# ChaissonLab/LRA

Hardware: AMD Instinct MI355X
Metric: aligned Gbp/s, 30 kb ONT vs GRCh38 (MapRead_lowacc end to end incl. SAM text), per job (higher is better)
Workload: dtype int32

## Files before the change

### lra_amd/csrc/sdp.h

```cpp
#pragma once
#include "common.h"
#include <vector>

namespace lra_sdp {

constexpr int LV = 18;
constexpr uint32_t NONE = 0xFFFFFFFFu;
constexpr int MAXALN = 16;
constexpr int PEN_TAB_WG = 4096, PEN_TAB_WAVE = 2048;
constexpr int TRACE_CAP = 2560;

struct PwlTab { long long stops[25]; float slope[25], inter[25]; int c1, c2; };

struct Ent { long long val; int b; float v; };
struct Node {
  uint32_t dBase;
  uint32_t nD, nE;
  int32_t last;
  uint32_t sTop, nBlk;
  uint32_t stkOff, blkOff;
  uint32_t stkCap, blkCap;
  long long eLast;
};

struct ReadArena { uint64_t base; uint32_t entOff, apOff, stkOff, visOff, blkPair, poolPair, poolPairs, edOff; };

struct PtArgs {
  uint64_t nc;
  const uint64_t* cluster_off; const uint64_t* c_start; const uint32_t* c_count; const int32_t* c_strand;
  const uint32_t* q; const uint32_t* t; const int32_t* len;
  const uint32_t* clusRead; const uint64_t* clusFragOff; const uint64_t* clusPtOff; const uint64_t* fragOff; const uint64_t* ptOff;
  const float* rate_in; float rate; int single;
  uint32_t* fq; uint32_t* ft; int32_t* flen; uint32_t* fcl; uint32_t* fai; float* fval; uint32_t* fprevNode; uint32_t* fprevInd; uint8_t* fflags;
  uint8_t* used; uint8_t* fstrand;
  const uint32_t* qe; const uint32_t* te; uint32_t* fqe; uint32_t* fte;
  uint64_t* key1; uint32_t* pay1; uint32_t* iq; uint32_t* it; uint8_t* ifl; uint32_t* ifr; uint32_t* ptRead;
};

struct BuildArgs {
  int r0, n;
  const uint32_t* order;
  const uint64_t* ptOff;
  const uint32_t* hq; const uint32_t* ht; const uint8_t* hfl; const uint32_t* h2; const uint64_t* key3; const uint32_t* pay3;
  uint32_t* scratch;
  uint32_t* cntEntries; uint32_t* cntNodes; uint32_t* cntD; uint32_t* cntV; uint32_t* cntRC;
  const ReadArena* ra;
  uint32_t* status;
  unsigned long long* stat;
};

struct ProcArgs {
  int r0, n;
  const uint32_t* order;
  const uint64_t* ptOff; const uint64_t* fragOff;
  const uint8_t* hfl; const uint32_t* hfr;
  const int32_t* flen; float* fval; uint32_t* fprevNode; uint32_t* fprevInd; uint8_t* fflags;
  const float* rate_in; float rate;
  const ReadArena* ra; uint32_t* poolUsed;
  uint32_t* status;
  PwlTab pwl;
  const short* penTab; int penN;
  int dbg;
  int wgNoRing;
  char* wgScratch; const uint64_t* wgOff;
  unsigned long long* stat;
};

struct TraceArgs {
  int r0, n, numAln, single; float alnthres;
  int boxes, globalK; const uint32_t* fqe; const uint32_t* fte; const int32_t* numAnchors; int32_t* chainNum;
  const uint64_t* fragOff; const uint64_t* read_off;
  const uint32_t* fq; const uint32_t* ft; const int32_t* flen; const uint32_t* fcl; const uint32_t* fai;
  const float* fval; const uint32_t* fpred; const uint8_t* fflags; const uint32_t* opay;
  uint8_t* used;
  const ReadArena* ra;
  uint32_t* nChains; uint64_t* chainStart; uint32_t* chainLen; uint32_t* chainBox; float* chainValue;
  uint32_t* ccl; uint32_t* can; uint8_t* clink; uint32_t* cq; uint32_t* ct; int32_t* clen; uint8_t* cstrand; const uint8_t* fstrand;
  const uint32_t* status;
};

namespace {
__device__ __forceinline__ void wave_sync() {
  __builtin_amdgcn_fence(__ATOMIC_RELEASE, "workgroup");
  __builtin_amdgcn_wave_barrier();
  __builtin_amdgcn_fence(__ATOMIC_ACQUIRE, "workgroup");
}
__device__ __forceinline__ int wave_incl_scan(int v, int lane) {
  (void)lane;
#define LRA_DPP_ADD(ctrl_, rmask_) v += __builtin_amdgcn_update_dpp(0, v, (ctrl_), (rmask_), 0xf, false)
  LRA_DPP_ADD(0x111, 0xf);
  LRA_DPP_ADD(0x112, 0xf);
  LRA_DPP_ADD(0x114, 0xf);
  LRA_DPP_ADD(0x118, 0xf);
  LRA_DPP_ADD(0x142, 0xa);
  LRA_DPP_ADD(0x143, 0xc);
#undef LRA_DPP_ADD
  return v;
}
__device__ __host__ inline uint32_t al256(uint64_t x) { return (uint32_t)((x + 255) & ~(uint64_t)255); }
__device__ __forceinline__ char* arena_ptr(uint64_t addr) { return (char*)(__attribute__((address_space(1))) char*)addr; }
}

#pragma GCC visibility push(hidden)
struct StatBuf {
  unsigned long long* d = nullptr;
  StatBuf() = default;
  StatBuf(const StatBuf&) = delete;
  StatBuf& operator=(const StatBuf&) = delete;
  ~StatBuf() { release(); }
  void alloc(size_t words, hipStream_t st) { release(); if (hipMalloc((void**)&d, words * 8) != hipSuccess) d = nullptr; else (void)hipMemsetAsync(d, 0, words * 8, st); }
  void release() { if (d) (void)hipFree(d); d = nullptr; }
};

struct Call {
  lra_ctx* ctx; hipStream_t st; const lra_sdp_opts* opts; lra_chain_result* out;
  int n_reads; size_t n1;
  const uint64_t* d_cluster_off; const uint64_t* d_c_start; const uint32_t* d_c_count; const int32_t* d_c_strand; const uint32_t* d_q; const uint32_t* d_t;
  const int32_t* d_len; const uint64_t* d_read_off; const float* d_rate; const uint32_t* d_qe; const uint32_t* d_te; const int32_t* d_num_anchors;
  bool boxes;
  PwlTab pw; short* d_penTab; int penN;
  lra_sort_opts sort;
  std::vector<uint64_t> h_off, h_frag, h_pt;
  uint64_t NC, NF, NP; size_t nslot;
  uint32_t* clusFragCnt; uint32_t* clusPtCnt; uint32_t* clusRead; uint64_t* clusFragOff; uint64_t* clusPtOff; uint64_t* fragOff; uint64_t* ptOff;
  uint32_t* status; uint32_t* nChains; uint64_t* chainStart; uint32_t* chainLen; float* chainValue; uint32_t* chainBox; int32_t* chainNum;
  uint32_t* fq; uint32_t* ft; int32_t* flen; uint32_t* fcl; uint32_t* fai; float* fval; uint32_t* fprevNode; uint32_t* fprevInd; uint32_t* ccl; uint32_t* can;
  uint8_t* fflags; uint8_t* used; uint8_t* clink; uint8_t* fstrand; uint8_t* cstrand; uint32_t* cq; uint32_t* ct; int32_t* clen; uint64_t* okey; uint32_t* fqe; uint32_t* fte;
  uint64_t* key1; uint64_t* key2; uint64_t* key3; uint32_t* pay1; uint32_t* pay2; uint32_t* pay3; uint32_t* iq; uint32_t* it; uint32_t* ifr; uint32_t* ptRead;
  uint32_t* hq; uint32_t* ht; uint32_t* hfr; uint32_t* spare; uint8_t* ifl; uint8_t* hfl; uint32_t* opay; uint32_t* fragRead;
  uint64_t totalEntries = 0;
};

struct Chunk {
  int r0, r1, nr; uint64_t cp;
  uint32_t* scratch; uint32_t* cntE; uint32_t* cntN; uint32_t* cntD; uint32_t* cntV; uint32_t* cntRC; uint32_t* order; uint32_t* order2; uint32_t* poolUsed;
  uint64_t* bytes; uint64_t* byteOff; ReadArena* ra;
  std::vector<uint32_t> h_orderAll, h_prev;
  BuildArgs ba; StatBuf buildStat;
  bool onePass;
  uint64_t totE = 0; uint32_t maxRC = 0;
  std::vector<uint32_t> h_status, h_sub;
  uint32_t* subOrder; int nsub;
  std::vector<uint64_t> woff;
};

struct Attempt {
  int att, shift, slot;
  const std::vector<uint32_t>* ordAtt;
  int nbig; bool forked, early;
  bool dbg;
  char* wsc = nullptr; uint64_t* dwoff = nullptr; uint32_t* d_maxLines = nullptr;
  uint64_t totB = 0; uint32_t bigLines = 0;
  ProcArgs pa;
  uint64_t dbgOff0 = 0; char* dbgBase = nullptr;
  hipEvent_t e0 = nullptr, e1 = nullptr;
};

void launch_cluster_counts(hipStream_t st, uint64_t nc, const uint32_t* c_count, uint32_t* fragCnt, uint32_t* ptCnt, int single);
void launch_read_offsets(hipStream_t st, int n_reads, const uint64_t* cluster_off, const uint64_t* clusFragOff, const uint64_t* clusPtOff, uint64_t* fragOff, uint64_t* ptOff,
                         uint32_t* clusRead, uint32_t* status, uint32_t* nChains);
void launch_points(hipStream_t st, const PtArgs& pa);
void launch_frag_read(hipStream_t st, int n_reads, const uint64_t* fragOff, uint32_t* fragRead);
void launch_gather(hipStream_t st, uint64_t np, const uint32_t* ptRead, const uint64_t* ptOff, const uint32_t* pay1, const uint32_t* iq, const uint32_t* it, const uint8_t* ifl,
                   const uint32_t* ifr, uint32_t* hq, uint32_t* ht, uint8_t* hfl, uint32_t* hfr, uint64_t* key2, uint32_t* pay2, uint64_t* key3, uint32_t* pay3);
void launch_reset_frags(hipStream_t st, int n, int r0, const uint32_t* order, const uint64_t* fragOff, const int32_t* flen, const float* rate_in, float rate, float* fval,
                        uint32_t* fprevNode, uint32_t* fprevInd, uint8_t* fflags, uint32_t* status);
void launch_pen_table(hipStream_t st, const PwlTab& pw, short* tab, int* bad);
void launch_arena_estimate(hipStream_t st, int n, int r0, const uint64_t* ptOff, float fE, float fN, uint32_t* cntE, uint32_t* cntN, uint32_t* cntD);
void launch_arena_sizes(hipStream_t st, int n, int r0, const uint64_t* ptOff, const uint32_t* cntE, const uint32_t* cntN, const uint32_t* cntD, ReadArena* ra, uint64_t* bytes,
                        const uint32_t* order, int shift);
void launch_arena_bases(hipStream_t st, int n, const uint64_t* byteOff, ReadArena* ra, const uint32_t* order, char* arena);
void launch_visit_clear(hipStream_t st, int n, const ReadArena* ra, const uint64_t* byteOff, const uint32_t* order);
void launch_big_lines(hipStream_t st, int n, int r0, const uint32_t* order, const uint64_t* ptOff, const uint32_t* hq, const uint32_t* ht, const uint32_t* h2, uint32_t* maxLines);
void launch_wg_builds(bool emit, hipStream_t st, const BuildArgs& ba, int n);
void launch_small_builds(bool emit, lra_ctx* ctx, const BuildArgs& ba, const uint32_t* d_order, const std::vector<uint32_t>& h_order, const uint64_t* h_pt, int from, int to);
void launch_process(hipStream_t st, const ProcArgs& pa, int n, bool stat);
void launch_process_wg(hipStream_t st, const ProcArgs& pa, int n, uint32_t lines, bool dbg);
void launch_valkeys(hipStream_t st, uint64_t f0, uint64_t n, const float* fval, const uint32_t* fragRead, const uint64_t* fragOff, uint64_t* okey, uint32_t* opay);
void launch_pred(hipStream_t st, uint64_t f0, uint64_t n, int r0, const uint32_t* fragRead, const uint32_t* fprevNode, const uint32_t* fprevInd, const uint32_t* status,
                 const ReadArena* ra, uint32_t* fpred);
void launch_trace(hipStream_t st, const TraceArgs& ta);
bool diag_dbg();
int diag_stat_level();
bool diag_build_stat();
int diag_dump(const Call& c);
void diag_ratios(const Call& c, const Chunk& k);
void diag_stat(const Call& c, const Attempt& a, int n, StatBuf& s);
void diag_dbg_begin(const Call& c, Attempt& a);
void diag_dbg_end(const Call& c, const Chunk& k, Attempt& a);
void diag_build_stat(const Call& c, Chunk& k);
#pragma GCC visibility pop

}
```

### lra_amd/csrc/sdp.hip

```cpp
#include "sdp.h"
#include "scan.h"
#include <algorithm>
#include <cmath>
#include <cstring>
#include <cstdlib>
#include <vector>

using namespace lra_sdp;

namespace {

inline size_t sz(size_t n, size_t elem) { return (n * elem + 255) / 256 * 256; }
inline char* take(char*& w, size_t n, size_t e) { char* p = w; w += sz(n, e); return p; }
#define SDP_TRY(call) do { const int rc__ = (call); if (rc__) return rc__; } while (0)

static long sdp_big_points(const lra_ctx* ctx, int mode) {
  if (const char* e = getenv("LRA_SDP_BIG_POINTS")) return atol(e);
  if (ctx->sdp_inner) return 1500;
  if (mode == 0) return 2500;
  return ctx->pipelined ? 14000 : 6000;
}

int pwl_table(Call& c) {
  lra_ctx* ctx = c.ctx; hipStream_t st = c.st; const lra_sdp_opts* opts = c.opts; PwlTab& pw = c.pw;
  {
    static const long long stv[25] = {0,    5,    10,   20,   40,   80,    100,   200,   300,   500,   1000,  2000, 3000,
                                      4000, 5000, 6000, 7000, 8000, 9000, 15000, 20000, 30000, 40000, 50000, 100000};
    float intercept = opts->gapopen, scalar = opts->gapextend, root = opts->gaproot, vals[25];
    for (int i = 0; i < 25; i++) { pw.stops[i] = stv[i]; pw.slope[i] = 0; pw.inter[i] = 0; }
    vals[0] = 0;
    for (int i = 1; i < 25; i++) { if (i <= 2) intercept = 0; vals[i] = intercept + scalar * std::pow((float)stv[i], 1 / root); }
    for (int i = 0; i < 24; i++) {
      float slope = (vals[i + 1] - vals[i]) / (stv[i + 1] - stv[i]);
      if (stv[i] <= 10) { pw.slope[i] = 0; pw.inter[i] = 0; }
      else { pw.slope[i] = slope; pw.inter[i] = vals[i] - stv[i] * slope + intercept; }
    }
    pw.c1 = opts->gapCeiling1; pw.c2 = opts->gapCeiling2;
  }
  c.d_penTab = (short*)lra_ensure(ctx, 190, PEN_TAB_WG * sizeof(short) + 64);
  c.penN = 0;
  if (c.d_penTab) {
    int* d_bad = (int*)(c.d_penTab + PEN_TAB_WG);
    LRA_HIP_CHECK(ctx, hipMemsetAsync(d_bad, 0, 4, st));
    launch_pen_table(st, pw, c.d_penTab, d_bad);
    int h_bad = 1;
    LRA_HIP_CHECK(ctx, hipMemcpyAsync(&h_bad, d_bad, 4, hipMemcpyDeviceToHost, st));
    LRA_HIP_CHECK(ctx, hipStreamSynchronize(st));
    if (!h_bad) c.penN = PEN_TAB_WG;
  }
  return LRA_OK;
}

int batch_buffers(Call& c) {
  lra_ctx* ctx = c.ctx; hipStream_t st = c.st; const lra_sdp_opts* opts = c.opts; lra_chain_result* out = c.out;
  const int n_reads = c.n_reads; const size_t n1 = c.n1;
  c.h_off.resize(n1);
  LRA_HIP_CHECK(ctx, hipMemcpyAsync(c.h_off.data(), c.d_cluster_off, n1 * 8, hipMemcpyDeviceToHost, st));
  LRA_HIP_CHECK(ctx, hipStreamSynchronize(st));
  const uint64_t NC = c.NC = c.h_off[n_reads];
  const size_t nslot = c.nslot = (size_t)n_reads * opts->NumAln;
  size_t needA = sz(NC + 1, 4) * 3 + sz(NC + 2, 8) * 2 + sz(n1, 8) * 2 + sz(n1, 4) * 2 + sz(nslot, 8) + sz(nslot, 4) * 3 + sz(4 * nslot, 4) + 4096;
  char* wa = (char*)lra_ensure(ctx, 7, needA);
  if (!wa) return LRA_ERR_NOMEM;
  c.clusFragCnt = (uint32_t*)take(wa, NC + 1, 4); c.clusPtCnt = (uint32_t*)take(wa, NC + 1, 4); c.clusRead = (uint32_t*)take(wa, NC + 1, 4);
  c.clusFragOff = (uint64_t*)take(wa, NC + 2, 8); c.clusPtOff = (uint64_t*)take(wa, NC + 2, 8);
  c.fragOff = (uint64_t*)take(wa, n1, 8); c.ptOff = (uint64_t*)take(wa, n1, 8);
  c.status = (uint32_t*)take(wa, n1, 4); c.nChains = (uint32_t*)take(wa, n1, 4);
  c.chainStart = (uint64_t*)take(wa, nslot, 8); c.chainLen = (uint32_t*)take(wa, nslot, 4); c.chainValue = (float*)take(wa, nslot, 4);
  c.chainBox = (uint32_t*)take(wa, 4 * nslot, 4);
  c.chainNum = (int32_t*)take(wa, nslot, 4);
  LRA_HIP_CHECK(ctx, hipMemsetAsync(c.chainLen, 0, nslot * 4, st));
  if (NC > 0) {
    lra_time_begin(ctx, ctx->sdp_inner ? "sdp_inner_points" : "sdp_points");
    launch_cluster_counts(st, NC, c.boxes ? nullptr : c.d_c_count, c.clusFragCnt, c.clusPtCnt, opts->mode == LRA_SDP_SINGLE_CLUSTER);
    lra_time_end(ctx);
  }
  SDP_TRY(lra_exclusive_scan<uint32_t>(ctx, (long)NC, c.clusFragCnt, c.clusFragOff));
  SDP_TRY(lra_exclusive_scan<uint32_t>(ctx, (long)NC, c.clusPtCnt, c.clusPtOff));
  launch_read_offsets(st, n_reads, c.d_cluster_off, c.clusFragOff, c.clusPtOff, c.fragOff, c.ptOff, c.clusRead, c.status, c.nChains);
  c.h_frag.resize(n1); c.h_pt.resize(n1);
  LRA_HIP_CHECK(ctx, hipMemcpyAsync(c.h_frag.data(), c.fragOff, n1 * 8, hipMemcpyDeviceToHost, st));
  LRA_HIP_CHECK(ctx, hipMemcpyAsync(c.h_pt.data(), c.ptOff, n1 * 8, hipMemcpyDeviceToHost, st));
  LRA_HIP_CHECK(ctx, hipStreamSynchronize(st));
  const uint64_t NF = c.NF = c.h_frag[n_reads], NP = c.NP = c.h_pt[n_reads];
  out->n_frags = NF; out->n_points = NP;
  size_t needF = sz(NF + 1, 4) * 16 + sz(2 * NF + 2, 4) + sz(NF + 1, 1) * 5 + sz(NF + 1, 8) * 2 + 4096;
  char* wf = (char*)lra_ensure(ctx, 8, needF);
  if (!wf) return LRA_ERR_NOMEM;
  c.fq = (uint32_t*)take(wf, NF + 1, 4); c.ft = (uint32_t*)take(wf, NF + 1, 4); c.flen = (int32_t*)take(wf, NF + 1, 4);
  c.fcl = (uint32_t*)take(wf, NF + 1, 4); c.fai = (uint32_t*)take(wf, NF + 1, 4); c.fval = (float*)take(wf, NF + 1, 4);
  c.fprevNode = (uint32_t*)take(wf, NF + 1, 4); c.fprevInd = (uint32_t*)take(wf, NF + 1, 4);
  c.ccl = (uint32_t*)take(wf, NF + 1, 4); c.can = (uint32_t*)take(wf, NF + 1, 4);
  c.fflags = (uint8_t*)take(wf, NF + 1, 1); c.used = (uint8_t*)take(wf, NF + 1, 1); c.clink = (uint8_t*)take(wf, NF + 1, 1);
  c.fstrand = (uint8_t*)take(wf, NF + 1, 1); c.cstrand = (uint8_t*)take(wf, NF + 1, 1);
  c.cq = (uint32_t*)take(wf, NF + 1, 4); c.ct = (uint32_t*)take(wf, NF + 1, 4); c.clen = (int32_t*)take(wf, NF + 1, 4);
  c.okey = (uint64_t*)take(wf, NF + 1, 8);
  c.fqe = (uint32_t*)take(wf, NF + 1, 4); c.fte = (uint32_t*)take(wf, NF + 1, 4);
  size_t needP = sz(NP + 1, 8) * 3 + sz(NP + 1, 4) * 11 + sz(NP + 1, 1) * 2 + sz(NF + 1, 4) * 2 + 4096;
  char* wp = (char*)lra_ensure(ctx, 9, needP);
  if (!wp) return LRA_ERR_NOMEM;
  c.key1 = (uint64_t*)take(wp, NP + 1, 8); c.key2 = (uint64_t*)take(wp, NP + 1, 8); c.key3 = (uint64_t*)take(wp, NP + 1, 8);
  c.pay1 = (uint32_t*)take(wp, NP + 1, 4); c.pay2 = (uint32_t*)take(wp, NP + 1, 4); c.pay3 = (uint32_t*)take(wp, NP + 1, 4);
  c.iq = (uint32_t*)take(wp, NP + 1, 4); c.it = (uint32_t*)take(wp, NP + 1, 4); c.ifr = (uint32_t*)take(wp, NP + 1, 4);
  c.ptRead = (uint32_t*)take(wp, NP + 1, 4);
  c.hq = (uint32_t*)take(wp, NP + 1, 4); c.ht = (uint32_t*)take(wp, NP + 1, 4); c.hfr = (uint32_t*)take(wp, NP + 1, 4);
  c.spare = (uint32_t*)take(wp, NP + 1, 4);
  c.ifl = (uint8_t*)take(wp, NP + 1, 1); c.hfl = (uint8_t*)take(wp, NP + 1, 1);
  c.opay = (uint32_t*)take(wp, NF + 1, 4); c.fragRead = (uint32_t*)take(wp, NF + 1, 4);
  out->d_n_chains = c.nChains; out->d_chain_start = c.chainStart; out->d_chain_len = c.chainLen; out->d_chain_box = c.chainBox; out->d_chain_value = c.chainValue;
  out->d_chain_cluster = c.ccl; out->d_chain_anchor = c.can; out->d_chain_link = c.clink; out->d_chain_q = c.cq; out->d_chain_t = c.ct; out->d_chain_alen = c.clen;
  out->d_chain_strand = c.cstrand; out->d_frag_off = c.fragOff; out->d_frag_val = c.fval; out->d_status = c.status;
  out->d_chain_num_anchors = c.boxes ? c.chainNum : nullptr;
  return LRA_OK;
}

void make_points(const Call& c) {
  lra_ctx* ctx = c.ctx; const lra_sdp_opts* opts = c.opts;
  PtArgs pa;
  pa.nc = c.NC; pa.cluster_off = c.d_cluster_off; pa.c_start = c.d_c_start; pa.c_count = c.d_c_count; pa.c_strand = c.d_c_strand; pa.q = c.d_q; pa.t = c.d_t; pa.len = c.d_len;
  pa.clusRead = c.clusRead; pa.clusFragOff = c.clusFragOff; pa.clusPtOff = c.clusPtOff; pa.fragOff = c.fragOff; pa.ptOff = c.ptOff; pa.rate_in = c.d_rate; pa.rate = opts->rate; pa.single = opts->mode == LRA_SDP_SINGLE_CLUSTER;
  pa.fq = c.fq; pa.ft = c.ft; pa.flen = c.flen; pa.fcl = c.fcl; pa.fai = c.fai; pa.fval = c.fval; pa.fprevNode = c.fprevNode; pa.fprevInd = c.fprevInd; pa.fflags = c.fflags; pa.used = c.used; pa.fstrand = c.fstrand;
  pa.qe = c.d_qe; pa.te = c.d_te; pa.fqe = c.fqe; pa.fte = c.fte;
  pa.key1 = c.key1; pa.pay1 = c.pay1; pa.iq = c.iq; pa.it = c.it; pa.ifl = c.ifl; pa.ifr = c.ifr; pa.ptRead = c.ptRead;
  lra_time_begin(ctx, ctx->sdp_inner ? "sdp_inner_points" : "sdp_points");
  launch_points(c.st, pa);
  launch_frag_read(c.st, c.n_reads, c.fragOff, c.fragRead);
  lra_time_end(ctx);
}

int sort_points(const Call& c) {
  lra_ctx* ctx = c.ctx; hipStream_t st = c.st; const int n_reads = c.n_reads; const uint64_t NP = c.NP;
  SDP_TRY(lra_sort_mostly_unique_batch(ctx, n_reads, c.ptOff, NP, c.key1, c.pay1, c.key3, c.pay3, 64, c.sort));
  lra_time_begin(ctx, ctx->sdp_inner ? "sdp_inner_points" : "sdp_points");
  launch_gather(st, NP, c.ptRead, c.ptOff, c.pay1, c.iq, c.it, c.ifl, c.ifr, c.hq, c.ht, c.hfl, c.hfr, c.key2, c.pay2, c.key3, c.pay3);
  lra_time_end(ctx);
  SDP_TRY(lra_sort_mostly_unique_batch(ctx, n_reads, c.ptOff, NP, c.key2, c.pay2, c.key1, c.pay1, 63, c.sort));
  lra_time_begin(ctx, c.sort.tag);
  const int rc = lra_segsort_pairs_scratch(ctx, c.key3, c.key1, c.pay3, c.pay1, NP, (uint64_t)n_reads, c.ptOff, c.ptOff + 1, 0, 42);
  lra_time_end(ctx);
  if (rc) return rc;
  LRA_HIP_CHECK(ctx, hipGetLastError());
  return LRA_OK;
}

int chunk_begin(const Call& c, Chunk& k) {
  lra_ctx* ctx = c.ctx; hipStream_t st = c.st; const std::vector<uint64_t>& h_pt = c.h_pt;
  const int r0 = k.r0, nr = k.nr; const uint64_t cp = k.cp;
  const size_t nr1 = (size_t)nr + 1;
  size_t needS = sz(34 * cp + 64 * (size_t)nr + 64, 4) + sz(nr1, 4) * 8 + sz(nr1 + 1, 8) * 3 + sz(nr1, sizeof(ReadArena)) + 4096;
  char* ws = (char*)lra_ensure(ctx, 10, needS);
  if (!ws) return LRA_ERR_NOMEM;
  k.scratch = (uint32_t*)take(ws, 34 * cp + 64 * (size_t)nr + 64, 4);
  k.cntE = (uint32_t*)take(ws, nr1, 4); k.cntN = (uint32_t*)take(ws, nr1, 4); k.cntD = (uint32_t*)take(ws, nr1, 4);
  k.cntV = (uint32_t*)take(ws, nr1, 4); k.cntRC = (uint32_t*)take(ws, nr1, 4); k.order = (uint32_t*)take(ws, nr1, 4); k.order2 = (uint32_t*)take(ws, nr1, 4); k.poolUsed = (uint32_t*)take(ws, nr1, 4);
  {
    std::vector<uint32_t> h_order(nr);
    uint64_t maxP = 0;
    for (int i = 0; i < nr; i++) maxP = std::max<uint64_t>(maxP, h_pt[r0 + i + 1] - h_pt[r0 + i]);
    if (maxP <= (uint64_t(1) << 24)) {
      std::vector<uint32_t> at(maxP + 2, 0);
      for (int i = 0; i < nr; i++) at[maxP - (h_pt[r0 + i + 1] - h_pt[r0 + i]) + 1]++;
      for (uint64_t v = 1; v <= maxP + 1; v++) at[v] += at[v - 1];
      for (int i = 0; i < nr; i++) h_order[at[maxP - (h_pt[r0 + i + 1] - h_pt[r0 + i])]++] = (uint32_t)i;
    } else {
      for (int i = 0; i < nr; i++) h_order[i] = (uint32_t)i;
      std::sort(h_order.begin(), h_order.end(), [&](uint32_t x, uint32_t y) {
        const uint64_t px = h_pt[r0 + x + 1] - h_pt[r0 + x], py = h_pt[r0 + y + 1] - h_pt[r0 + y];
        return px != py ? px > py : x < y;
      });
    }
    LRA_HIP_CHECK(ctx, hipMemcpyAsync(k.order, h_order.data(), (size_t)nr * 4, hipMemcpyHostToDevice, st));
    LRA_HIP_CHECK(ctx, hipStreamSynchronize(st));
    k.h_orderAll = h_order;
  }
  take(ws, nr1 + 1, 8);
  k.bytes = (uint64_t*)take(ws, nr1 + 1, 8); k.byteOff = (uint64_t*)take(ws, nr1 + 1, 8);
  k.ra = (ReadArena*)take(ws, nr1, sizeof(ReadArena));
  BuildArgs& ba = k.ba;
  memset(&ba, 0, sizeof ba);
  ba.r0 = r0; ba.n = nr; ba.ptOff = c.ptOff; ba.hq = c.hq; ba.ht = c.ht; ba.hfl = c.hfl; ba.h2 = c.pay2; ba.key3 = c.key1; ba.pay3 = c.pay1; ba.scratch = k.scratch;
  ba.cntEntries = k.cntE; ba.cntNodes = k.cntN; ba.cntD = k.cntD; ba.cntV = k.cntV; ba.cntRC = k.cntRC; ba.status = c.status; ba.order = k.order; ba.stat = nullptr;
  if (diag_build_stat()) { k.buildStat.alloc(16, st); ba.stat = k.buildStat.d; }
  k.h_status.assign(nr, 0);
  k.subOrder = k.order; k.nsub = nr;
  return LRA_OK;
}

void count_pass(const Call& c, const Chunk& k, const uint32_t* d_ord, const std::vector<uint32_t>& h_ord, int n) {
  lra_ctx* ctx = c.ctx; hipStream_t st = c.st; const lra_sdp_opts* opts = c.opts; const std::vector<uint64_t>& h_pt = c.h_pt; const int r0 = k.r0;
  lra_time_begin(ctx, ctx->sdp_inner ? "sdp_inner_build_count" : "sdp_build_count");
  const long big_pts = sdp_big_points(ctx, opts->mode);
  int nb0 = 0;
  while (nb0 < n && (long)(h_pt[r0 + h_ord[nb0] + 1] - h_pt[r0 + h_ord[nb0]]) >= big_pts) nb0++;
  const bool forked = nb0 > 0 && n > nb0;
  BuildArgs bc = k.ba; bc.order = d_ord; bc.n = n;
  if (nb0 > 0) launch_wg_builds(false, forked ? lra_side_fork(ctx) : st, bc, nb0);
  if (n > nb0) launch_small_builds(false, ctx, bc, d_ord, h_ord, h_pt.data() + r0, nb0, n);
  if (forked) lra_side_join(ctx);
  lra_time_end(ctx);
}

int read_rc(const Call& c, Chunk& k) {
  lra_ctx* ctx = c.ctx; hipStream_t st = c.st; const int nr = k.nr;
  std::vector<uint32_t> h_rc(nr), h_e(nr);
  LRA_HIP_CHECK(ctx, hipMemcpyAsync(h_rc.data(), k.cntRC, (size_t)nr * 4, hipMemcpyDeviceToHost, st));
  LRA_HIP_CHECK(ctx, hipMemcpyAsync(h_e.data(), k.onePass ? k.cntV : k.cntE, (size_t)nr * 4, hipMemcpyDeviceToHost, st));
  LRA_HIP_CHECK(ctx, hipStreamSynchronize(st));
  k.maxRC = 0; k.totE = 0;
  for (uint32_t v : h_rc) k.maxRC = std::max(k.maxRC, v);
  for (uint32_t v : h_e) k.totE += v;
  return LRA_OK;
}

int chunk_sizes(const Call& c, Chunk& k) {
  const lra_sdp_opts* opts = c.opts; const int nr = k.nr;
  const bool onePassEnv = !(getenv("LRA_SDP_ONEPASS") && getenv("LRA_SDP_ONEPASS")[0] == '0');
  k.onePass = onePassEnv && !getenv("LRA_SDP_RATIOS");
  if (!k.onePass) { count_pass(c, k, k.order, k.h_orderAll, nr); SDP_TRY(read_rc(c, k)); }
  else {
    float fE = opts->mode == 0 ? 10.0f : 8.5f, fN = 2.0f;
    if (const char* e = getenv("LRA_SDP_ESTIMATE")) { float x = 0, y = 0; if (sscanf(e, "%f,%f", &x, &y) == 2 && x > 0 && y > 0) { fE = x; fN = y; } }
    launch_arena_estimate(c.st, nr, k.r0, c.ptOff, fE, fN, k.cntE, k.cntN, k.cntD);
  }
  diag_ratios(c, k);
  return LRA_OK;
}

void pick_large_reads(const Call& c, const Chunk& k, Attempt& a) {
  lra_ctx* ctx = c.ctx; const lra_sdp_opts* opts = c.opts; const std::vector<uint64_t>& h_pt = c.h_pt; const std::vector<uint32_t>& ordAtt = *a.ordAtt;
  const int r0 = k.r0, nsub = k.nsub, att = a.att; const bool onePass = k.onePass, dbg = a.dbg;
  int nbig = 0;
  {
    const long big_pts = sdp_big_points(ctx, opts->mode);
    const int maxBigAll = ctx->pipelined ? ctx->num_cu : (1 << 30);
    const int maxBig = (opts->mode == 0 && !ctx->sdp_inner) ? std::min(maxBigAll, 512) : maxBigAll;
    while (nbig < nsub && nbig < maxBig && (long)(h_pt[r0 + ordAtt[nbig] + 1] - h_pt[r0 + ordAtt[nbig]]) >= big_pts) nbig++;
  }
  const bool forked = nbig > 0 && nsub > nbig;
  const bool bigFirstEnv = !(getenv("LRA_SDP_BIG_FIRST") && getenv("LRA_SDP_BIG_FIRST")[0] == '0');
  const bool early = bigFirstEnv && att == 0 && onePass && forked && !dbg;
  a.nbig = nbig; a.forked = forked; a.early = early;
}

int arena_layout(const Call& c, Chunk& k, Attempt& a) {
  lra_ctx* ctx = c.ctx; hipStream_t st = c.st; const std::vector<uint64_t>& h_frag = c.h_frag; const std::vector<uint64_t>& h_pt = c.h_pt;
  const std::vector<uint32_t>& ordAtt = *a.ordAtt; std::vector<uint64_t>& woff = k.woff;
  const int r0 = k.r0, nsub = k.nsub, nbig = a.nbig;
  woff.assign((size_t)nbig + 1, 0);
  if (nbig > 0) {
    for (int i = 0; i < nbig; i++) {
      const uint64_t rdx = (uint64_t)r0 + ordAtt[i];
      const uint64_t Fr = h_frag[rdx + 1] - h_frag[rdx], Pr = h_pt[rdx + 1] - h_pt[rdx];
      woff[i + 1] = woff[i] + ((36 * Fr + 4 * Pr + 64 + 8 + 256 * 8 + 255) & ~(uint64_t)255);
    }
    a.wsc = (char*)lra_ensure(ctx, 177, woff[nbig] + 256);
    a.dwoff = (uint64_t*)lra_ensure(ctx, 178, ((size_t)nbig + 4) * 8);
    if (!a.wsc || !a.dwoff) return LRA_ERR_NOMEM;
    a.d_maxLines = (uint32_t*)(a.dwoff + nbig + 2);
    LRA_HIP_CHECK(ctx, hipMemcpyAsync(a.dwoff, woff.data(), ((size_t)nbig + 1) * 8, hipMemcpyHostToDevice, st));
    if (a.early) {
      LRA_HIP_CHECK(ctx, hipMemsetAsync(a.d_maxLines, 0, 4, st));
      launch_big_lines(st, nbig, r0, k.subOrder, c.ptOff, c.hq, c.ht, c.pay2, a.d_maxLines);
    }
  }
  launch_arena_sizes(st, nsub, r0, c.ptOff, k.cntE, k.cntN, k.cntD, k.ra, k.bytes, k.subOrder, a.shift);
  SDP_TRY(lra_exclusive_scan<uint64_t>(ctx, nsub, k.bytes, k.byteOff));
  LRA_HIP_CHECK(ctx, hipMemcpyAsync(&a.totB, k.byteOff + nsub, 8, hipMemcpyDeviceToHost, st));
  if (a.early) LRA_HIP_CHECK(ctx, hipMemcpyAsync(&a.bigLines, a.d_maxLines, 4, hipMemcpyDeviceToHost, st));
  return LRA_OK;
}

int emit_builds(const Call& c, Chunk& k, Attempt& a) {
  lra_ctx* ctx = c.ctx; hipStream_t st = c.st; const std::vector<uint32_t>& ordAtt = *a.ordAtt; BuildArgs& ba = k.ba;
  const uint64_t* h_pt0 = c.h_pt.data() + k.r0;
  const int nsub = k.nsub, nbig = a.nbig;
  if (a.early) LRA_HIP_CHECK(ctx, hipMemsetAsync(k.poolUsed, 0, (size_t)k.nr * 4, st));
  lra_time_begin(ctx, ctx->sdp_inner ? "sdp_inner_build" : "sdp_build");
  launch_visit_clear(st, nsub, k.ra, k.byteOff, k.subOrder);
  ba.ra = k.ra; ba.order = k.subOrder;
  if (a.early) {
    hipStream_t ws = lra_side_fork(ctx);
    if (ws == st) {
      launch_wg_builds(true, st, ba, nbig);
      launch_small_builds(true, ctx, ba, k.subOrder, ordAtt, h_pt0, nbig, nsub);
      launch_process_wg(st, a.pa, nbig, a.bigLines, a.dbg);
    } else {
      launch_wg_builds(true, ws, ba, nbig);
      if (!ctx->ev_mid) (void)hipEventCreateWithFlags(&ctx->ev_mid, hipEventDisableTiming);
      if (ctx->ev_mid) { (void)hipEventRecord(ctx->ev_mid, ws); (void)hipStreamWaitEvent(st, ctx->ev_mid, 0); }
      lra_time_begin(ctx, ctx->sdp_inner ? "sdp_inner_process_wg" : "sdp_process_wg", ws);
      launch_process_wg(ws, a.pa, nbig, a.bigLines, a.dbg);
      lra_time_end(ctx, ws);
      launch_small_builds(true, ctx, ba, k.subOrder, ordAtt, h_pt0, nbig, nsub);
    }
  } else {
    if (nbig > 0) launch_wg_builds(true, a.forked ? lra_side_fork(ctx) : st, ba, nbig);
    if (nsub > nbig) launch_small_builds(true, ctx, ba, k.subOrder, ordAtt, h_pt0, nbig, nsub);
    if (a.forked) lra_side_join(ctx);
  }
  lra_time_end(ctx);
  if (k.onePass && a.att == 0) SDP_TRY(read_rc(c, k));
  return LRA_OK;
}

int process_points(const Call& c, Chunk& k, Attempt& a) {
  lra_ctx* ctx = c.ctx; hipStream_t st = c.st;
  const int nsub = k.nsub, nbig = a.nbig;
  if (a.att > 0)
    launch_reset_frags(st, nsub, k.r0, k.subOrder, c.fragOff, c.flen, c.d_rate, c.opts->rate, c.fval, c.fprevNode, c.fprevInd, c.fflags, c.status);
  if (!a.early) LRA_HIP_CHECK(ctx, hipMemsetAsync(k.poolUsed, 0, (size_t)k.nr * 4, st));
  diag_dbg_begin(c, a);
  lra_time_begin(ctx, ctx->sdp_inner ? "sdp_inner_process" : "sdp_process");
  if (nbig > 0 && !a.early) launch_process_wg(a.forked ? lra_side_fork(ctx) : st, a.pa, nbig, k.maxRC, a.dbg);
  const int statEnv = diag_stat_level();
  StatBuf stat;
  if (nsub > nbig) {
    ProcArgs pb = a.pa; pb.order = k.subOrder + nbig; pb.n = nsub - nbig; pb.stat = nullptr;
    if (statEnv > 0) stat.alloc(40, st);
    if (stat.d) { pb.stat = stat.d; pb.dbg = statEnv; }
    launch_process(st, pb, nsub - nbig, stat.d != nullptr);
  }
  if (a.forked) lra_side_join(ctx);
  lra_time_end(ctx);
  diag_stat(c, a, nsub - nbig, stat);
  diag_dbg_end(c, k, a);
  return LRA_OK;
}

int collect_outgrown(const Call& c, Chunk& k, const Attempt& a) {
  lra_ctx* ctx = c.ctx; hipStream_t st = c.st; const int nr = k.nr;
  LRA_HIP_CHECK(ctx, hipMemcpyAsync(k.h_status.data(), c.status + k.r0, (size_t)nr * 4, hipMemcpyDeviceToHost, st));
  LRA_HIP_CHECK(ctx, hipStreamSynchronize(st));
  k.h_sub.clear();
  for (int i = 0; i < k.nsub; i++) { const uint32_t rr = (*a.ordAtt)[i]; if (k.h_status[rr] & LRA_ST_CAPACITY) k.h_sub.push_back(rr); }
  k.nsub = (int)k.h_sub.size();
  if (k.nsub == 0) return LRA_OK;
  k.h_prev = k.h_sub;
  LRA_HIP_CHECK(ctx, hipMemcpyAsync(k.order2, k.h_sub.data(), (size_t)k.nsub * 4, hipMemcpyHostToDevice, st));
  LRA_HIP_CHECK(ctx, hipStreamSynchronize(st));
  k.subOrder = k.order2;
  return LRA_OK;
}

int attempt(const Call& c, Chunk& k, int att) {
  lra_ctx* ctx = c.ctx; hipStream_t st = c.st;
  Attempt a;
  a.att = att; a.shift = 3 * att; a.slot = att == 0 ? 12 : 21 + att;
  if (k.onePass && att == 1) count_pass(c, k, k.subOrder, k.h_prev, k.nsub);
  a.dbg = diag_dbg();
  a.ordAtt = att == 0 ? &k.h_orderAll : &k.h_prev;
  pick_large_reads(c, k, a);
  {
    const int rc = arena_layout(c, k, a);
    const hipError_t e = hipStreamSynchronize(st);
    if (rc) return rc;
    LRA_HIP_CHECK(ctx, e);
  }
  char* arena = (char*)lra_ensure(ctx, a.slot, a.totB + 4096);
  if (!arena) return LRA_ERR_NOMEM;
  launch_arena_bases(st, k.nsub, k.byteOff, k.ra, k.subOrder, arena);
  ProcArgs& pa = a.pa;
  pa.wgScratch = a.wsc; pa.wgOff = a.dwoff; pa.dbg = (a.dbg && a.nbig > 0) ? 1 : 0; { const char* e = getenv("LRA_SDP_WG_RING"); pa.wgNoRing = (e && e[0] == '0') ? 1 : 0; }
  if (a.nbig > 0) {
    const uint64_t rd0 = (uint64_t)k.r0 + (*a.ordAtt)[0];
    a.dbgOff0 = k.woff[0] + 36 * (c.h_frag[rd0 + 1] - c.h_frag[rd0]) + 4 * (c.h_pt[rd0 + 1] - c.h_pt[rd0]); a.dbgBase = a.wsc;
  }
  pa.r0 = k.r0; pa.n = k.nsub; pa.order = k.subOrder; pa.ptOff = c.ptOff; pa.fragOff = c.fragOff; pa.hfl = c.hfl; pa.hfr = c.hfr; pa.flen = c.flen; pa.fval = c.fval;
  pa.fprevNode = c.fprevNode; pa.fprevInd = c.fprevInd; pa.fflags = c.fflags; pa.rate_in = c.d_rate; pa.rate = c.opts->rate; pa.ra = k.ra;
  pa.status = c.status; pa.pwl = c.pw; pa.poolUsed = k.poolUsed; pa.penTab = c.d_penTab; pa.penN = c.penN;
  SDP_TRY(emit_builds(c, k, a));
  SDP_TRY(process_points(c, k, a));
  if (att == 2) return LRA_OK;
  return collect_outgrown(c, k, a);
}

int trace_chains(const Call& c, const Chunk& k) {
  lra_ctx* ctx = c.ctx; hipStream_t st = c.st; const lra_sdp_opts* opts = c.opts; const int r0 = k.r0, nr = k.nr;
  const uint64_t cf0 = c.h_frag[r0], cfn = c.h_frag[k.r1] - c.h_frag[r0];
  if (cfn == 0) return LRA_OK;
    lra_time_begin(ctx, ctx->sdp_inner ? "sdp_inner_trace" : "sdp_trace");
    const bool needOrder = opts->mode != LRA_SDP_SINGLE_CLUSTER;
  if (needOrder) launch_valkeys(st, cf0, cfn, c.fval, c.fragRead, c.fragOff, c.okey, c.opay);
  launch_pred(st, cf0, cfn, r0, c.fragRead, c.fprevNode, c.fprevInd, c.status, k.ra, c.spare);
  lra_time_end(ctx);
  if (needOrder) SDP_TRY(lra_sort_exact_batch(ctx, nr, c.fragOff + r0, c.okey, c.opay, c.sort));
  TraceArgs ta;
  ta.r0 = r0; ta.n = nr; ta.numAln = opts->NumAln; ta.single = opts->mode == LRA_SDP_SINGLE_CLUSTER; ta.alnthres = opts->alnthres; ta.fragOff = c.fragOff; ta.read_off = c.d_read_off; ta.fq = c.fq; ta.ft = c.ft;
  ta.flen = c.flen; ta.fcl = c.fcl; ta.fai = c.fai; ta.fval = c.fval; ta.fpred = c.spare; ta.fflags = c.fflags; ta.opay = c.opay; ta.used = c.used;
  ta.ra = k.ra; ta.nChains = c.nChains; ta.chainStart = c.chainStart; ta.chainLen = c.chainLen;
  ta.chainBox = c.chainBox; ta.chainValue = c.chainValue; ta.ccl = c.ccl; ta.can = c.can; ta.clink = c.clink; ta.status = c.status;
  ta.cq = c.cq; ta.ct = c.ct; ta.clen = c.clen; ta.cstrand = c.cstrand; ta.fstrand = c.fstrand;
  ta.boxes = c.boxes; ta.globalK = opts->globalK; ta.fqe = c.fqe; ta.fte = c.fte; ta.numAnchors = c.d_num_anchors; ta.chainNum = c.chainNum;
  lra_time_begin(ctx, ctx->sdp_inner ? "sdp_inner_trace" : "sdp_trace");
  launch_trace(st, ta);
  lra_time_end(ctx);
  return LRA_OK;
}

int sdp_run(lra_ctx* ctx, int n_reads, const uint64_t* d_cluster_off, const uint64_t* d_c_start, const uint32_t* d_c_count,
            const int32_t* d_c_strand, const uint32_t* d_q, const uint32_t* d_t, const int32_t* d_len, const uint64_t* d_read_off,
            const float* d_rate, const lra_sdp_opts* opts, lra_chain_result* out, const uint32_t* d_qe, const uint32_t* d_te,
            const int32_t* d_num_anchors) {
  if (!ctx || !out || !opts || n_reads < 0) return LRA_ERR_INVALID;
  if (opts->NumAln < 1 || opts->NumAln > MAXALN) return lra_set_err(ctx, LRA_ERR_INVALID, "NumAln must be 1..%d", MAXALN);
  memset(out, 0, sizeof *out);
  out->n_reads = n_reads; out->num_aln = opts->NumAln;
  if (n_reads == 0) return LRA_OK;
  LRA_HIP_CHECK(ctx, hipSetDevice(ctx->device));
  Call c;
  c.ctx = ctx; c.st = ctx->stream; c.opts = opts; c.out = out; c.n_reads = n_reads; c.n1 = (size_t)n_reads + 1;
  c.d_cluster_off = d_cluster_off; c.d_c_start = d_c_start; c.d_c_count = d_c_count; c.d_c_strand = d_c_strand; c.d_q = d_q; c.d_t = d_t; c.d_len = d_len;
  c.d_read_off = d_read_off; c.d_rate = d_rate; c.d_qe = d_qe; c.d_te = d_te; c.d_num_anchors = d_num_anchors; c.boxes = d_qe != nullptr;
  c.sort = ctx->sdp_inner ? lra_sort_opts{"sdp_inner_sort", "sdp_inner_sort_fallback", true} : lra_sort_opts{"sdp_sort", "sdp_sort_fallback", true};
  SDP_TRY(pwl_table(c));
  SDP_TRY(batch_buffers(c));
  if (c.NF == 0) { LRA_HIP_CHECK(ctx, hipStreamSynchronize(c.st)); return LRA_OK; }
  make_points(c);
  SDP_TRY(diag_dump(c));
  SDP_TRY(sort_points(c));
  constexpr uint64_t chunkPts = 96ull << 20;
  const std::vector<uint64_t>& h_pt = c.h_pt;
  for (int r0 = 0; r0 < n_reads;) {
    int r1 = r0 + 1;
    while (r1 < n_reads && h_pt[r1 + 1] - h_pt[r0] <= chunkPts) r1++;
    Chunk k;
    k.r0 = r0; k.r1 = r1; k.nr = r1 - r0; k.cp = h_pt[r1] - h_pt[r0];
    r0 = r1;
    if (k.cp == 0) continue;
    SDP_TRY(chunk_begin(c, k));
    SDP_TRY(chunk_sizes(c, k));
    for (int att = 0; att < 3 && k.nsub > 0; att++) SDP_TRY(attempt(c, k, att));
    diag_build_stat(c, k);
    if (k.onePass) SDP_TRY(read_rc(c, k));
    c.totalEntries += k.totE;
    SDP_TRY(trace_chains(c, k));
    LRA_HIP_CHECK(ctx, hipGetLastError());
  }
  out->n_subproblem_entries = c.totalEntries;
  LRA_HIP_CHECK(ctx, hipStreamSynchronize(c.st));
  LRA_HIP_CHECK(ctx, hipGetLastError());
  return LRA_OK;
}

}

extern "C" int lra_sparse_dp_batch(lra_ctx* ctx, int n_reads, const uint64_t* d_cluster_off, const uint64_t* d_c_start, const uint32_t* d_c_count,
                                   const int32_t* d_c_strand, const uint32_t* d_q, const uint32_t* d_t, const int32_t* d_len,
                                   const uint64_t* d_read_off, const float* d_rate, const lra_sdp_opts* opts, lra_chain_result* out) {
  if (opts && opts->mode != LRA_SDP_CLUSTERS && opts->mode != LRA_SDP_SINGLE_CLUSTER) return lra_set_err(ctx, LRA_ERR_INVALID, "mode must be 0 or 1");
  return sdp_run(ctx, n_reads, d_cluster_off, d_c_start, d_c_count, d_c_strand, d_q, d_t, d_len, d_read_off, d_rate, opts, out, nullptr, nullptr, nullptr);
}

extern "C" int lra_sparse_dp_boxes_batch(lra_ctx* ctx, int n_reads, const uint64_t* d_box_off, const uint32_t* d_qs, const uint32_t* d_qe,
                                         const uint32_t* d_ts, const uint32_t* d_te, const int32_t* d_strand, const int32_t* d_val,
                                         const int32_t* d_num_anchors, const uint64_t* d_read_off, const float* d_rate, const lra_sdp_opts* opts,
                                         lra_chain_result* out) {
  if (!opts || !d_qe || !d_te) return LRA_ERR_INVALID;
  lra_sdp_opts o = *opts;
  o.mode = LRA_SDP_CLUSTERS;
  return sdp_run(ctx, n_reads, d_box_off, nullptr, nullptr, d_strand, d_qs, d_ts, d_val, d_read_off, d_rate, &o, out, d_qe, d_te, d_num_anchors);
}
```

### lra_amd/csrc/sdp_build.hip

```cpp
#include "sdp.h"
#include <type_traits>

using namespace lra_sdp;

namespace {

template <int NW>
__device__ __forceinline__ int blk_incl_scan(int v, int lane, int wave, int* s_w, int& total) {
  const int inc = wave_incl_scan(v, lane);
  if (NW == 1) { total = __builtin_amdgcn_readlane(inc, 63); return inc; }
  if (lane == 63) s_w[wave] = inc;
  __syncthreads();
  int pre = 0, tot = 0;
#pragma unroll
  for (int w = 0; w < NW; w++) { const int x = s_w[w]; tot += x; if (w < wave) pre += x; }
  __syncthreads();
  total = tot;
  return inc + pre;
}
template <bool EMIT, int NW, int MODE = 0, int OCC = 8, bool BSTAT = false>
__global__ void __launch_bounds__(64 * NW, NW == 1 ? OCC : 1) sdp_build(BuildArgs a) {
  constexpr int NT = 64 * NW;
  constexpr bool LDSV = MODE == 1, NARROW = MODE != 0;
  using IT = typename std::conditional<NARROW, uint16_t, uint32_t>::type;
  using DT = typename std::conditional<NARROW, uint32_t, long long>::type;
  constexpr IT INONE = (IT)~(IT)0;
  extern __shared__ __attribute__((aligned(16))) char dyn_lds[];
  __shared__ int s_w[4][NW == 1 ? 1 : NW];
  __shared__ unsigned long long s_bt[BSTAT ? 8 : 1];
  unsigned long long btPrev = 0;
  constexpr bool bstat = BSTAT;
  if (bstat) { if (threadIdx.x < 8) s_bt[threadIdx.x] = 0; btPrev = __builtin_amdgcn_s_memtime(); }
#define BTICK(k_) do { if (bstat) { const unsigned long long t__ = __builtin_amdgcn_s_memtime(); if (threadIdx.x == 0) s_bt[k_] += t__ - btPrev; btPrev = t__; } } while (0)
  const int rr = (int)a.order[blockIdx.x], r = a.r0 + rr, tid = threadIdx.x, lane = tid & 63, wave = tid >> 6;
  auto SYNC = [&]() { if (NW == 1) wave_sync(); else __syncthreads(); };
  const uint64_t p0 = a.ptOff[r], pc0 = a.ptOff[a.r0];
  const int P = (int)(a.ptOff[r + 1] - p0);
  if (P == 0) { if (tid == 0) { if (!EMIT) { a.cntEntries[rr] = 0; a.cntNodes[rr] = 0; a.cntD[rr] = 0; } a.cntV[rr] = 0; a.cntRC[rr] = 0; } return; }
  const uint32_t* hq = a.hq + p0; const uint32_t* ht = a.ht + p0; const uint32_t* h2 = a.h2 + p0;
  const uint64_t* key3 = a.key3 + p0; const uint32_t* pay3 = a.pay3 + p0;
  uint32_t* S = a.scratch + 34 * (p0 - pc0) + 64 * (uint64_t)rr;
  const int NCAP = P + 2;
  uint32_t* tbl = S + 8 * P + 2;
  uint32_t* tmp = tbl + 12 * NCAP;
  IT* eb_ = LDSV ? (IT*)dyn_lds : (IT*)S;
  IT* rowOf = eb_; IT* colOf = rowOf + P;
  IT* lp = colOf + P;
  IT* ln = lp + 2 * P;
  IT* pf = ln + 2 * P;
  IT* ph = pf + P + 1;
  IT* ll = NARROW ? ph + P + 1 : (IT*)(tmp + 8 * NCAP);
  DT* ld = LDSV ? (DT*)(dyn_lds + ((((size_t)(10 * P + 2) * sizeof(IT)) + 7) & ~(size_t)7)) : NARROW ? (DT*)(tmp + 8 * NCAP) : (DT*)(ll + 2 * P);
  auto LN = [&](int idx) -> uint32_t { const IT v = ln[idx]; return v == INONE ? NONE : (uint32_t)v; };
#define TB(c, f, k) tbl[((c) * 6 + (f)) * NCAP + (k)]
#define TM(f, k) tmp[(f) * NCAP + (k)]
  enum { F_LS, F_LE, F_SB, F_SE, F_EB, F_EE };
  enum { T_C1S, T_C1E, T_ND, T_NE, T_CH0, T_CH1, T_BASE, T_GID };
  int R = 0, C = 0;
  for (int i0 = 0; i0 < P; i0 += NT) {
    const int i = i0 + tid;
    const int head = (i < P) && (i == 0 || hq[i] != hq[i - 1]);
    int tot; const int inc = blk_incl_scan<NW>(head, lane, wave, s_w[0], tot);
    if (i < P) rowOf[i] = R + inc - 1;
    R += tot;
  }
  for (int i0 = 0; i0 < P; i0 += NT) {
    const int i = i0 + tid;
    const int head = (i < P) && (i == 0 || ht[h2[i]] != ht[h2[i - 1]]);
    int tot; const int inc = blk_incl_scan<NW>(head, lane, wave, s_w[0], tot);
    if (i < P) colOf[h2[i]] = C + inc - 1;
    C += tot;
  }
  int cOff[5];
  {
    int c0 = 0, c1 = 0, c2 = 0, c3 = 0;
    for (int i = tid; i < P; i += NT) { const int cl = (int)(key3[i] >> 40); c0 += cl == 0; c1 += cl == 1; c2 += cl == 2; c3 += cl == 3; }
    for (int o = 32; o > 0; o >>= 1) { c0 += __shfl_xor(c0, o); c1 += __shfl_xor(c1, o); c2 += __shfl_xor(c2, o); c3 += __shfl_xor(c3, o); }
    if (NW > 1) {
      if (lane == 0) { s_w[0][wave] = c0; s_w[1][wave] = c1; s_w[2][wave] = c2; s_w[3][wave] = c3; }
      __syncthreads();
      c0 = c1 = c2 = c3 = 0;
      for (int w = 0; w < NW; w++) { c0 += s_w[0][w]; c1 += s_w[1][w]; c2 += s_w[2][w]; c3 += s_w[3][w]; }
      __syncthreads();
    }
    c0 = __builtin_amdgcn_readfirstlane(c0); c1 = __builtin_amdgcn_readfirstlane(c1); c2 = __builtin_amdgcn_readfirstlane(c2);
    cOff[0] = 0; cOff[1] = c0; cOff[2] = c0 + c1; cOff[3] = c0 + c1 + c2; cOff[4] = P;
  }
  SYNC();
  BTICK(0);
  uint32_t nEntries = 0, nNodesTot = 0, sumD = 0, nVisits = 0;
  Node* nodesR = nullptr; Ent* entR = nullptr; uint32_t* apR = nullptr; int2* stkR = nullptr; uint2* visR = nullptr; long long* edR = nullptr;
  uint32_t blkPair = 0;
  if (EMIT) {
    const ReadArena A = a.ra[rr];
    char* b = arena_ptr(A.base);
    blkPair = A.blkPair;
    nodesR = (Node*)b; entR = (Ent*)(b + A.entOff); apR = (uint32_t*)(b + A.apOff); stkR = (int2*)(b + A.stkOff); visR = (uint2*)(b + A.visOff);
    edR = (long long*)(b + A.edOff);
  }
  bool overflow = false, outgrown = false;
  const uint64_t capE = EMIT ? a.cntEntries[rr] : 0, capN = EMIT ? a.cntNodes[rr] : 0, capD = EMIT ? a.cntD[rr] : 0;
  for (int fam = 0; fam < 4 && !outgrown; fam++) {
    const bool col = fam & 1, back = fam >= 2, desc = (fam == 1 || fam == 2), swapped = (fam == 3);
    const IT* lineOf = col ? colOf : rowOf;
    const int nLines = col ? C : R;
    const int sc = back ? 2 : 0;
    const int nS = cOff[sc + 1] - cOff[sc], nEn = cOff[sc + 2] - cOff[sc + 1], Pf = nS + nEn;
    if (nS == 0 || nEn == 0) continue;
    const int fam2 = fam & 1;
    const int dSide = swapped ? 1 : 0, eSide = swapped ? 0 : 1;
    for (int i = tid; i < Pf; i += NT) {
      const uint32_t pos = pay3[cOff[sc] + i];
      lp[i] = (IT)pos; ln[i] = 0; ll[i] = lineOf[pos];
      ld[i] = (DT)(back ? (long long)ht[pos] + hq[pos] : (long long)ht[pos] - hq[pos]);
    }
    if (tid == 0) { TB(0, F_LS, 0) = 0; TB(0, F_LE, 0) = nLines; TB(0, F_SB, 0) = 0; TB(0, F_SE, 0) = nS; TB(0, F_EB, 0) = nS; TB(0, F_EE, 0) = Pf; }
    int nNodes = 1, cur = 0;
    SYNC();
    BTICK(7);
    for (int level = 0; nNodes > 0 && !outgrown; level++) {
      if (level >= LV) { overflow = true; break; }
      const int nxt = cur ^ 1;
      IT* lpc = lp + cur * P; IT* lpn = lp + nxt * P;
      IT* llc = ll + cur * P; IT* lln = ll + nxt * P;
      DT* ldc = ld + (size_t)cur * P; DT* ldn = ld + (size_t)nxt * P;
      {
        int carry = 0;
        constexpr int UA = 4;
        for (int i0 = 0; i0 < Pf; i0 += UA * NT) {
          uint32_t kk[UA]; uint32_t ss[UA], ee[UA]; IT lv[UA]; int ff[UA];
#pragma unroll
          for (int u = 0; u < UA; u++) { const int i = i0 + u * NT + tid; kk[u] = i < Pf ? LN(i) : NONE; lv[u] = i < Pf ? llc[i] : (IT)0; }
#pragma unroll
          for (int u = 0; u < UA; u++) { ss[u] = 0; ee[u] = 0; if (kk[u] != NONE) { ss[u] = TB(cur, F_LS, kk[u]); ee[u] = TB(cur, F_LE, kk[u]); } }
#pragma unroll
          for (int u = 0; u < UA; u++) ff[u] = kk[u] == NONE ? 0 : (ee[u] - ss[u] > 1) ? (lv[u] < ((ss[u] + ee[u]) >> 1)) : 1;
#pragma unroll
          for (int u = 0; u < UA; u++) {
            const int i = i0 + u * NT + tid;
            if (i0 + u * NT >= Pf) break;
            int tot; const int inc = blk_incl_scan<NW>(ff[u], lane, wave, s_w[0], tot);
            if (i < Pf) pf[i] = (IT)(carry + inc - ff[u]);
            carry += tot;
          }
        }
        if (tid == 0) pf[Pf] = (IT)carry;
      }
      SYNC();
      BTICK(1);
      for (int k = tid; k < nNodes; k += NT) {
        TM(T_C1S, k) = (uint32_t)pf[TB(cur, F_SE, k)] - (uint32_t)pf[TB(cur, F_SB, k)];
        TM(T_C1E, k) = (uint32_t)pf[TB(cur, F_EE, k)] - (uint32_t)pf[TB(cur, F_EB, k)];
      }
      SYNC();
      {
        constexpr int UC = 2;
        for (int i0 = 0; i0 < Pf; i0 += UC * NT) {
          uint32_t kk[UC], pi0[UC], pi1[UC], sb[UC], c1[UC], psb[UC]; IT vlp[UC], vll[UC]; DT vld[UC];
#pragma unroll
          for (int u = 0; u < UC; u++) {
            const int i = i0 + u * NT + tid;
            kk[u] = NONE; pi0[u] = 0; pi1[u] = 0; vlp[u] = 0; vll[u] = 0; vld[u] = 0;
            if (i < Pf) { kk[u] = LN(i); pi0[u] = (uint32_t)pf[i]; pi1[u] = (uint32_t)pf[i + 1]; vlp[u] = lpc[i]; vll[u] = llc[i]; vld[u] = ldc[i]; }
          }
#pragma unroll
          for (int u = 0; u < UC; u++) {
            const int i = i0 + u * NT + tid;
            const bool isS = i < nS;
            sb[u] = 0; c1[u] = 0;
            if (kk[u] != NONE) { sb[u] = isS ? TB(cur, F_SB, kk[u]) : TB(cur, F_EB, kk[u]); c1[u] = isS ? TM(T_C1S, kk[u]) : TM(T_C1E, kk[u]); }
          }
#pragma unroll
          for (int u = 0; u < UC; u++) psb[u] = kk[u] != NONE ? (uint32_t)pf[sb[u]] : 0;
#pragma unroll
          for (int u = 0; u < UC; u++) {
            const int i = i0 + u * NT + tid;
            if (i >= Pf) continue;
            if (kk[u] == NONE) { ln[P + i] = INONE; continue; }
            const uint32_t rank1 = pi0[u] - psb[u];
            const uint32_t first = pi1[u] - pi0[u];
            const uint32_t np_ = first ? sb[u] + rank1 : sb[u] + c1[u] + ((uint32_t)i - sb[u] - rank1);
            lpn[np_] = vlp[u]; lln[np_] = vll[u]; ldn[np_] = vld[u];
            ln[P + np_] = (IT)(2 * kk[u] + (first ? 0 : 1));
          }
        }
      }
      SYNC();
      BTICK(2);
      {
        int carry = 0;
        constexpr int UD = NW == 1 ? 4 : 2;
        for (int j0 = 0; j0 < Pf; j0 += UD * NT) {
          uint32_t k2v[UD], le[UD], ls[UD], bg[UD], c1[UD]; DT d0[UD], d1[UD]; int hd[UD];
#pragma unroll
          for (int u = 0; u < UD; u++) {
            const int j = j0 + u * NT + tid;
            k2v[u] = NONE; d0[u] = 0; d1[u] = 0;
            if (j < Pf) { k2v[u] = LN(P + j); d0[u] = ldn[j]; d1[u] = j > 0 ? ldn[j - 1] : ldn[j]; }
          }
#pragma unroll
          for (int u = 0; u < UD; u++) {
            const int j = j0 + u * NT + tid;
            const bool isS = j < nS;
            le[u] = 0; ls[u] = 0; bg[u] = 0; c1[u] = 0;
            if (k2v[u] != NONE) {
              const uint32_t k = k2v[u] >> 1;
              le[u] = TB(cur, F_LE, k); ls[u] = TB(cur, F_LS, k); bg[u] = isS ? TB(cur, F_SB, k) : TB(cur, F_EB, k); c1[u] = isS ? TM(T_C1S, k) : TM(T_C1E, k);
            }
          }
#pragma unroll
          for (int u = 0; u < UD; u++) {
            const int j = j0 + u * NT + tid;
            hd[u] = 0;
            if (k2v[u] != NONE) {
              const uint32_t side = k2v[u] & 1;
              const bool isS = j < nS;
              const bool leaf = le[u] - ls[u] == 1;
              const bool in = leaf || (int)side == (isS ? eSide : dSide);
              if (in) {
                uint32_t beg = bg[u];
                if (!leaf && side == 1) beg += c1[u];
                hd[u] = ((uint32_t)j == beg) ? 1 : (d0[u] != d1[u]);
              }
            }
          }
#pragma unroll
          for (int u = 0; u < UD; u++) {
            const int j = j0 + u * NT + tid;
            if (j0 + u * NT >= Pf) break;
            int tot; const int inc = blk_incl_scan<NW>(hd[u], lane, wave, s_w[0], tot);
            if (j < Pf) ph[j] = (IT)(carry + inc - hd[u]);
            carry += tot;
          }
        }
        if (tid == 0) ph[Pf] = (IT)carry;
      }
      SYNC();
      BTICK(3);
      int nNext = 0;
      for (int k0 = 0; k0 < nNodes; k0 += NT) {
        const int k = k0 + tid;
        uint32_t nD = 0, nE = 0, act0 = 0, act1 = 0, full = 0;
        uint32_t ls = 0, le = 0, sb = 0, se = 0, eb = 0, ee = 0, c1S = 0, c1E = 0;
        bool leaf = false;
        if (k < nNodes) {
          ls = TB(cur, F_LS, k); le = TB(cur, F_LE, k); sb = TB(cur, F_SB, k); se = TB(cur, F_SE, k); eb = TB(cur, F_EB, k); ee = TB(cur, F_EE, k);
          c1S = TM(T_C1S, k); c1E = TM(T_C1E, k);
          leaf = le - ls == 1;
          uint32_t dB, dE, eB, eE;
          if (leaf) { dB = eb; dE = ee; eB = sb; eE = se; }
          else {
            dB = dSide == 0 ? eb : eb + c1E; dE = dSide == 0 ? eb + c1E : ee;
            eB = eSide == 0 ? sb : sb + c1S; eE = eSide == 0 ? sb + c1S : se;
          }
          nD = (uint32_t)ph[dE] - (uint32_t)ph[dB]; nE = (uint32_t)ph[eE] - (uint32_t)ph[eB];
          full = nD > 0 && nE > 0;
          if (!leaf) {
            const bool goD = nD > 0, goE = nE > 0;
            if (dSide == 0) { act0 = goD; act1 = goE; } else { act1 = goD; act0 = goE; }
          }
        }
        int totF, totEnt, totD, totC;
        const int incF = blk_incl_scan<NW>((int)full, lane, wave, s_w[0], totF), incEnt = blk_incl_scan<NW>((int)(full ? nD + nE : 0), lane, wave, s_w[1], totEnt),
                  incD = blk_incl_scan<NW>((int)(full ? nD : 0), lane, wave, s_w[2], totD), incC = blk_incl_scan<NW>((int)(act0 + act1), lane, wave, s_w[3], totC);
        if (EMIT && ((uint64_t)nNodesTot + totF > capN || (uint64_t)nEntries + totEnt > capE || (uint64_t)sumD + totD > capD)) { outgrown = true; break; }
        if (k < nNodes) {
          const uint32_t gid = nNodesTot + incF - full, base = nEntries + incEnt - (full ? nD + nE : 0), dpre = sumD + incD - (full ? nD : 0);
          TM(T_ND, k) = nD; TM(T_NE, k) = nE; TM(T_GID, k) = full ? gid : NONE; TM(T_BASE, k) = base;
          uint32_t ci = nNext + incC - (act0 + act1);
          const uint32_t med = (ls + le) >> 1;
          TM(T_CH0, k) = NONE; TM(T_CH1, k) = NONE;
          if (act0) { TM(T_CH0, k) = ci; TB(nxt, F_LS, ci) = ls; TB(nxt, F_LE, ci) = med; TB(nxt, F_SB, ci) = sb; TB(nxt, F_SE, ci) = sb + c1S;
                      TB(nxt, F_EB, ci) = eb; TB(nxt, F_EE, ci) = eb + c1E; ci++; }
          if (act1) { TM(T_CH1, k) = ci; TB(nxt, F_LS, ci) = med; TB(nxt, F_LE, ci) = le; TB(nxt, F_SB, ci) = sb + c1S; TB(nxt, F_SE, ci) = se;
                      TB(nxt, F_EB, ci) = eb + c1E; TB(nxt, F_EE, ci) = ee; }
          if (EMIT && full) {
            Node nd;
            nd.dBase = base; nd.nD = nD; nd.nE = nE; nd.last = -1; nd.sTop = 1; nd.nBlk = 0;
            nd.stkOff = 2 * dpre + 4 * gid; nd.blkOff = blkPair + 2 * base + 8 * gid; nd.stkCap = 2 * nD + 4; nd.blkCap = 2 * (nD + nE) + 8;
            nd.eLast = 0;
            nodesR[gid] = nd;
            stkR[nd.stkOff] = make_int2(-1, (int)nE + 1);
          }
        }
        nNodesTot += totF; nEntries += totEnt; sumD += totD; nNext += totC;
      }
      if (outgrown) break;
      SYNC();
      BTICK(4);
      {
        constexpr int UF = 2;
        for (int j0 = 0; j0 < Pf; j0 += UF * NT) {
          uint32_t k2v[UF], le[UF], ls[UF], ch[UF], gidv[UF], bg[UF], c1[UF], nNE[UF], nND[UF], bs[UF], p0v[UF], p1v[UF], pbg[UF], posv[UF], tq[UF], tt[UF];
#pragma unroll
          for (int u = 0; u < UF; u++) {
            const int j = j0 + u * NT + tid;
            k2v[u] = NONE; p0v[u] = 0; p1v[u] = 0; posv[u] = 0;
            if (j < Pf) { k2v[u] = LN(P + j); if (EMIT) { p0v[u] = (uint32_t)ph[j]; p1v[u] = (uint32_t)ph[j + 1]; posv[u] = lpn[j]; } }
          }
#pragma unroll
          for (int u = 0; u < UF; u++) {
            const int j = j0 + u * NT + tid;
            const bool isS = j < nS;
            le[u] = 0; ls[u] = 0; ch[u] = 0; gidv[u] = NONE; bg[u] = 0; c1[u] = 0; nNE[u] = 0; nND[u] = 0; bs[u] = 0; tq[u] = 0; tt[u] = 0;
            if (k2v[u] != NONE) {
              const uint32_t k = k2v[u] >> 1, side = k2v[u] & 1;
              le[u] = TB(cur, F_LE, k); ls[u] = TB(cur, F_LS, k); ch[u] = side == 0 ? TM(T_CH0, k) : TM(T_CH1, k); gidv[u] = TM(T_GID, k);
              if (EMIT) {
                bg[u] = isS ? TB(cur, F_SB, k) : TB(cur, F_EB, k); c1[u] = isS ? TM(T_C1S, k) : TM(T_C1E, k);
                nNE[u] = TM(T_NE, k); nND[u] = TM(T_ND, k); bs[u] = TM(T_BASE, k);
                tq[u] = hq[posv[u]]; tt[u] = ht[posv[u]];
              }
            }
          }
#pragma unroll
          for (int u = 0; u < UF; u++) {
            pbg[u] = 0;
            if (EMIT && k2v[u] != NONE) {
              const uint32_t side = k2v[u] & 1;
              const bool leaf = le[u] - ls[u] == 1;
              uint32_t beg = bg[u];
              if (!leaf && side == 1) beg += c1[u];
              bg[u] = beg;
              pbg[u] = (uint32_t)ph[beg];
            }
          }
#pragma unroll
          for (int u = 0; u < UF; u++) {
            const int j = j0 + u * NT + tid;
            if (j >= Pf) continue;
            if (k2v[u] == NONE) { ln[j] = INONE; continue; }
            const uint32_t side = k2v[u] & 1;
            const bool leaf = le[u] - ls[u] == 1;
            ln[j] = (IT)(leaf ? NONE : ch[u]);
            const uint32_t gid = gidv[u];
            const bool isS = j < nS;
            const bool in = leaf || (int)side == (isS ? eSide : dSide);
            if (in && gid != NONE) {
              if (!EMIT) nVisits++;
              else {
                const uint32_t head = p1v[u] - p0v[u];
                const uint32_t grp = p0v[u] - pbg[u] + head - 1;
                const uint32_t n = isS ? nNE[u] : nND[u];
                const uint32_t idx = desc ? n - 1 - grp : grp;
                const uint32_t ent = bs[u] + (isS ? nND[u] + idx : idx);
                const uint32_t pos = posv[u];
                if (head) {
                  const long long dgv = back ? (long long)tt[u] + tq[u] : (long long)tt[u] - tq[u];
                  entR[ent].val = dgv;
                  if (isS && idx == n - 1) nodesR[gid].eLast = dgv;
                }
                visR[(uint64_t)pos * (2 * LV) + fam2 * LV + level] = make_uint2(gid, idx);
              }
            }
          }
        }
      }
      SYNC();
      BTICK(5);
      if (EMIT) {
        constexpr int UG = 2;
        for (int j0 = 0; j0 < Pf; j0 += UG * NT) {
          uint32_t k2v[UG], gidv[UG], le[UG], ls[UG], bg[UG], c1[UG], nDv[UG], nEv[UG], bs[UG], p0v[UG], p1v[UG], pbg[UG];
          bool on[UG];
#pragma unroll
          for (int u = 0; u < UG; u++) {
            const int j = j0 + u * NT + tid;
            k2v[u] = NONE; p0v[u] = 0; p1v[u] = 0;
            if (j < Pf) { k2v[u] = LN(P + j); p0v[u] = (uint32_t)ph[j]; p1v[u] = (uint32_t)ph[j + 1]; }
          }
#pragma unroll
          for (int u = 0; u < UG; u++) {
            const int j = j0 + u * NT + tid;
            const bool isS = j < nS;
            gidv[u] = NONE; le[u] = 0; ls[u] = 0; bg[u] = 0; c1[u] = 0; nDv[u] = 0; nEv[u] = 0; bs[u] = 0;
            if (k2v[u] != NONE && p1v[u] != p0v[u]) {
              const uint32_t k = k2v[u] >> 1;
              gidv[u] = TM(T_GID, k); le[u] = TB(cur, F_LE, k); ls[u] = TB(cur, F_LS, k);
              bg[u] = isS ? TB(cur, F_SB, k) : TB(cur, F_EB, k); c1[u] = isS ? TM(T_C1S, k) : TM(T_C1E, k);
              nDv[u] = TM(T_ND, k); nEv[u] = TM(T_NE, k); bs[u] = TM(T_BASE, k);
            }
          }
#pragma unroll
          for (int u = 0; u < UG; u++) {
            const int j = j0 + u * NT + tid;
            const bool isS = j < nS;
            const uint32_t side = k2v[u] & 1;
            const bool leaf = le[u] - ls[u] == 1;
            on[u] = k2v[u] != NONE && p1v[u] != p0v[u] && gidv[u] != NONE && (leaf || (int)side == (isS ? eSide : dSide));
            pbg[u] = 0;
            if (on[u]) { uint32_t beg = bg[u]; if (!leaf && side == 1) beg += c1[u]; pbg[u] = (uint32_t)ph[beg]; }
          }
          uint32_t entv[UG], mv[UG], lo[UG], cnt[UG]; long long xv[UG]; const Ent* opp[UG];
#pragma unroll
          for (int u = 0; u < UG; u++) {
            const int j = j0 + u * NT + tid;
            const bool isS = j < nS;
            const uint32_t grp = p0v[u] - pbg[u];
            const uint32_t n = isS ? nEv[u] : nDv[u];
            const uint32_t idx = desc ? n - 1 - grp : grp;
            entv[u] = bs[u] + (isS ? nDv[u] + idx : idx);
            opp[u] = entR + bs[u] + (isS ? 0 : nDv[u]);
            mv[u] = isS ? nDv[u] : nEv[u];
            xv[u] = on[u] ? entR[entv[u]].val : 0;
            lo[u] = 0; cnt[u] = on[u] ? mv[u] : 0;
          }
          while (true) {
            bool any = false;
#pragma unroll
            for (int u = 0; u < UG; u++) any |= cnt[u] > 0;
            if (!any) break;
            long long vM[UG], vL[UG], vR[UG];
#pragma unroll
            for (int u = 0; u < UG; u++) {
              const uint32_t step = cnt[u] >> 1, it = lo[u] + step, cntT = cnt[u] > 0 ? cnt[u] - step - 1 : 0;
              vM[u] = cnt[u] > 0 ? opp[u][it].val : 0;
              vL[u] = step > 0 ? opp[u][lo[u] + (step >> 1)].val : 0;
              vR[u] = cntT > 0 ? opp[u][it + 1 + (cntT >> 1)].val : 0;
            }
#pragma unroll
            for (int u = 0; u < UG; u++) {
              if (cnt[u] == 0) continue;
              const bool isS = j0 + u * NT + tid < nS;
              auto go = [&](long long v) { return isS ? (desc ? v > xv[u] : v <= xv[u]) : (desc ? v >= xv[u] : v < xv[u]); };
              const uint32_t step = cnt[u] >> 1, it = lo[u] + step;
              if (go(vM[u])) {
                lo[u] = it + 1; cnt[u] -= step + 1;
                if (cnt[u] > 0) { const uint32_t s2 = cnt[u] >> 1; if (go(vR[u])) { lo[u] += s2 + 1; cnt[u] -= s2 + 1; } else cnt[u] = s2; }
              } else {
                cnt[u] = step;
                if (cnt[u] > 0) { const uint32_t s2 = cnt[u] >> 1; if (go(vL[u])) { lo[u] += s2 + 1; cnt[u] -= s2 + 1; } else cnt[u] = s2; }
              }
            }
          }
#pragma unroll
          for (int u = 0; u < UG; u++) {
            if (!on[u]) continue;
            const bool isS = j0 + u * NT + tid < nS;
            const uint32_t ent = entv[u], m = mv[u];
            entR[ent].b = isS ? (int32_t)lo[u] - 1 : (lo[u] == m ? -1 : (int32_t)lo[u]);
            if (!isS) edR[ent] = lo[u] == m ? 0 : opp[u][lo[u]].val;
            entR[ent].v = 0.f; apR[ent] = 0;
          }
        }
      }
      nNodes = nNext; cur = nxt;
      SYNC();
      BTICK(6);
    }
  }
  if (bstat && tid == 0) { for (int k = 0; k < 8; k++) atomicAdd(a.stat + k, s_bt[k]); atomicAdd(a.stat + 8, (unsigned long long)P); }
  for (int o = 32; o > 0; o >>= 1) nVisits += __shfl_xor(nVisits, o);
  if (NW > 1) {
    if (lane == 0) s_w[0][wave] = (int)nVisits;
    __syncthreads();
    nVisits = 0;
    for (int w = 0; w < NW; w++) nVisits += (uint32_t)s_w[0][w];
  }
  if (tid == 0) {
    if (!EMIT) { a.cntEntries[rr] = nEntries; a.cntNodes[rr] = nNodesTot; a.cntD[rr] = sumD; a.cntV[rr] = nVisits; a.cntRC[rr] = (uint32_t)max(R, C); }
    else { a.cntV[rr] = nEntries; a.cntRC[rr] = (uint32_t)max(R, C); }
    if (overflow) atomicOr(&a.status[r], (uint32_t)LRA_ST_RANGE);
    if (outgrown) atomicOr(&a.status[r], (uint32_t)LRA_ST_CAPACITY);
  }
#undef TB
#undef TM
#undef BTICK
}

template <bool EMIT>
void small_builds(lra_ctx* ctx, const BuildArgs& ba, const uint32_t* d_order, const std::vector<uint32_t>& h_order, const uint64_t* h_pt, int from, int to) {
  hipStream_t st = ctx->stream;
  auto pts = [&](int i) { return (long)(h_pt[h_order[i] + 1] - h_pt[h_order[i]]); };
  int at = from;
  const long caps[3] = {512, 256, 128};
  int cut[4];
  for (int c = 0; c < 3; c++) { while (at < to && pts(at) > caps[c]) at++; cut[c] = at; }
  cut[3] = to;
  if (cut[0] > from) {
    int mid = from;
    while (mid < cut[0] && pts(mid) >= 16384) mid++;
    if (mid > from) { BuildArgs bb = ba; bb.order = d_order + from; hipLaunchKernelGGL((sdp_build<EMIT, 1, 0>), dim3(mid - from), dim3(64), 0, st, bb); }
    if (cut[0] > mid) {
      BuildArgs bb = ba; bb.order = d_order + mid;
      const bool occ6 = ctx->pipelined;
      if (bb.stat) { if (occ6) hipLaunchKernelGGL((sdp_build<EMIT, 1, 2, 6, true>), dim3(cut[0] - mid), dim3(64), 0, st, bb); else hipLaunchKernelGGL((sdp_build<EMIT, 1, 2, 8, true>), dim3(cut[0] - mid), dim3(64), 0, st, bb); }
      else if (occ6) hipLaunchKernelGGL((sdp_build<EMIT, 1, 2, 6>), dim3(cut[0] - mid), dim3(64), 0, st, bb);
      else hipLaunchKernelGGL((sdp_build<EMIT, 1, 2>), dim3(cut[0] - mid), dim3(64), 0, st, bb);
    }
  }
  for (int c = 0; c < 3; c++) {
    const int n = cut[c + 1] - cut[c];
    if (n <= 0) continue;
    BuildArgs bb = ba; bb.order = d_order + cut[c];
    hipLaunchKernelGGL((sdp_build<EMIT, 1, 1>), dim3(n), dim3(64), (size_t)(28 * caps[c] + 32), st, bb);
  }
}

}

namespace lra_sdp {

void launch_wg_builds(bool emit, hipStream_t st, const BuildArgs& ba, int n) {
  if (emit) hipLaunchKernelGGL((sdp_build<true, 16>), dim3(n), dim3(1024), 0, st, ba);
  else hipLaunchKernelGGL((sdp_build<false, 16>), dim3(n), dim3(1024), 0, st, ba);
}
void launch_small_builds(bool emit, lra_ctx* ctx, const BuildArgs& ba, const uint32_t* d_order, const std::vector<uint32_t>& h_order, const uint64_t* h_pt, int from, int to) {
  if (emit) small_builds<true>(ctx, ba, d_order, h_order, h_pt, from, to);
  else small_builds<false>(ctx, ba, d_order, h_order, h_pt, from, to);
}

}
```

### lra_amd/csrc/sdp_points.hip

```cpp
#include <algorithm>
#include "sdp_process.h"

using namespace lra_sdp;

namespace {

__global__ void k_arena_sizes(int n, int r0, const uint64_t* __restrict__ ptOff, const uint32_t* __restrict__ cntE, const uint32_t* __restrict__ cntN,
                              const uint32_t* __restrict__ cntD, ReadArena* ra, uint64_t* bytes, const uint32_t* __restrict__ order, int shift) {
  int b = blockIdx.x * blockDim.x + threadIdx.x;
  if (b >= n) return;
  const int rr = (int)order[b];
  const uint64_t E = cntE[rr], N = cntN[rr], D = cntD[rr], P = ptOff[r0 + rr + 1] - ptOff[r0 + rr];
  ReadArena a;
  a.base = 0;
  uint64_t o = al256(N * sizeof(Node));
  a.entOff = (uint32_t)o; o = al256(o + E * sizeof(Ent));
  a.apOff = (uint32_t)o; o = al256(o + E * 4);
  a.edOff = (uint32_t)o; o = al256(o + E * 8);
  const uint64_t stkPairs = 2 * D + 4 * N + 2, blkPairs = 2 * E + 8 * N + 2, poolPairs = (2 * E + 4096) << shift;
  a.stkOff = (uint32_t)o; a.blkPair = (uint32_t)stkPairs; a.poolPair = (uint32_t)(stkPairs + blkPairs); a.poolPairs = (uint32_t)poolPairs;
  o = al256(o + (stkPairs + blkPairs + poolPairs) * 8);
  a.visOff = (uint32_t)o; o = al256(o + P * 2 * LV * sizeof(uint2));
  ra[rr] = a;
  bytes[b] = o;
}
__global__ void k_arena_estimate(int n, int r0, const uint64_t* __restrict__ ptOff, float fE, float fN, uint32_t* cntE, uint32_t* cntN, uint32_t* cntD) {
  int rr = blockIdx.x * blockDim.x + threadIdx.x;
  if (rr >= n) return;
  const uint64_t P = ptOff[r0 + rr + 1] - ptOff[r0 + rr];
  const uint64_t E = (uint64_t)(fE * (float)P) + 64, N = (uint64_t)(fN * (float)P) + 64;
  cntE[rr] = (uint32_t)std::min<uint64_t>(E, 0xFFFFFFFFull); cntN[rr] = (uint32_t)std::min<uint64_t>(N, 0xFFFFFFFFull); cntD[rr] = (uint32_t)std::min<uint64_t>(E * 6 / 10 + 64, 0xFFFFFFFFull);
}
__global__ void k_arena_bases(int n, const uint64_t* __restrict__ byteOff, ReadArena* ra, const uint32_t* __restrict__ order, char* arena) {
  int b = blockIdx.x * blockDim.x + threadIdx.x;
  if (b < n) ra[order[b]].base = (uint64_t)(uintptr_t)(arena + byteOff[b]);
}
__global__ void k_visit_clear(const ReadArena* __restrict__ ra, const uint64_t* __restrict__ byteOff, const uint32_t* __restrict__ order) {
  const int b = blockIdx.x;
  const ReadArena A = ra[order[b]];
  uint4* p = (uint4*)(arena_ptr(A.base) + A.visOff);
  const uint64_t n = (byteOff[b + 1] - byteOff[b] - A.visOff) / 16;
  for (uint64_t i = threadIdx.x; i < n; i += blockDim.x) p[i] = make_uint4(NONE, NONE, NONE, NONE);
}

__global__ void k_big_lines(int r0, const uint32_t* __restrict__ order, const uint64_t* __restrict__ ptOff, const uint32_t* __restrict__ hq, const uint32_t* __restrict__ ht,
                            const uint32_t* __restrict__ h2, uint32_t* maxLines) {
  const int r = r0 + (int)order[blockIdx.x];
  const uint64_t p0 = ptOff[r];
  const int P = (int)(ptOff[r + 1] - p0);
  const uint32_t* q = hq + p0; const uint32_t* t = ht + p0; const uint32_t* c = h2 + p0;
  uint32_t R = 0, C = 0;
  for (int i = threadIdx.x; i < P; i += blockDim.x) { R += (i == 0 || q[i] != q[i - 1]); C += (i == 0 || t[c[i]] != t[c[i - 1]]); }
  for (int o = 32; o > 0; o >>= 1) { R += __shfl_xor(R, o); C += __shfl_xor(C, o); }
  __shared__ uint32_t sR, sC;
  if (threadIdx.x == 0) { sR = 0; sC = 0; }
  __syncthreads();
  if ((threadIdx.x & 63) == 0) { atomicAdd(&sR, R); atomicAdd(&sC, C); }
  __syncthreads();
  if (threadIdx.x == 0) atomicMax(maxLines, max(sR, sC));
}

__global__ void k_cluster_counts(uint64_t nc, const uint32_t* __restrict__ c_count, uint32_t* fragCnt, uint32_t* ptCnt, int single) {
  uint64_t c = (uint64_t)blockIdx.x * blockDim.x + threadIdx.x;
  if (c >= nc) return;
  if (!c_count) { fragCnt[c] = 1; ptCnt[c] = 4; return; }
  uint32_t n = c_count[c];
  fragCnt[c] = n;
  ptCnt[c] = 2 * n + (single ? 0 : 2 * (n == 0 ? 0 : n == 1 ? 1 : 2));
}

__global__ void k_read_offsets(int n_reads, const uint64_t* __restrict__ cluster_off, const uint64_t* __restrict__ clusFragOff,
                               const uint64_t* __restrict__ clusPtOff, uint64_t* fragOff, uint64_t* ptOff, uint32_t* clusRead,
                               uint32_t* status, uint32_t* nChains) {
  int r = blockIdx.x * blockDim.x + threadIdx.x;
  if (r > n_reads) return;
  fragOff[r] = clusFragOff[cluster_off[r]];
  ptOff[r] = clusPtOff[cluster_off[r]];
  if (r < n_reads) {
    for (uint64_t c = cluster_off[r]; c < cluster_off[r + 1]; c++) clusRead[c] = r;
    status[r] = 0; nChains[r] = 0;
  }
}

__global__ void k_points(PtArgs a) {
  const bool boxMode = a.qe != nullptr;
  const uint64_t gtid = (uint64_t)blockIdx.x * blockDim.x + threadIdx.x;
  const uint64_t c = boxMode ? gtid : (gtid >> 6);
  const uint32_t lane = threadIdx.x & 63;
  if (c >= a.nc) return;
  const uint32_t r = a.clusRead[c];
  const int strand = a.c_strand[c];
  uint64_t g = a.clusFragOff[c], p = a.clusPtOff[c];
  const uint64_t f0 = a.fragOff[r], p0 = a.ptOff[r];
  const uint32_t cl = (uint32_t)(c - a.cluster_off[r]);
  const float rate = a.rate_in ? a.rate_in[r] : a.rate;
  if (a.qe) {
    const uint32_t qs = a.q[c], ts = a.t[c], qe = a.qe[c], te = a.te[c];
    const int val = a.len[c];
    a.fq[g] = qs; a.ft[g] = ts; a.fqe[g] = qe; a.fte[g] = te; a.flen[g] = val; a.fcl[g] = cl; a.fai[g] = 0;
    a.fval[g] = val * rate;
    a.fprevNode[g] = NONE; a.fprevInd[g] = NONE; a.fflags[g] = 3; a.used[g] = 0; a.fstrand[g] = (uint8_t)(strand != 0);
    const uint32_t lf = (uint32_t)(g - f0);
    for (int k = 0; k < 4; k++, p++) {
      const uint8_t ind = (k & 1) ? 0 : 1, inv = k < 2 ? 1 : 0;
      const uint32_t pq = ind ? qs + 1 : qe - 1;
      const uint32_t pt = (k == 0 || k == 3) ? ts + 1 : te - 1;
      a.key1[p] = ((uint64_t)pq << 33) | ((uint64_t)pt << 1) | ind;
      a.pay1[p] = (uint32_t)(p - p0);
      a.iq[p] = pq; a.it[p] = pt; a.ifl[p] = (uint8_t)(ind | (inv << 1)); a.ifr[p] = lf; a.ptRead[p] = r;
    }
    return;
  }
  const uint32_t n = a.c_count[c];
  const uint64_t src = a.c_start[c];
  const uint64_t g0 = g, pc0 = p;
  for (uint32_t i = lane; i < n; i += 64) {
    g = g0 + i; p = pc0 + 2 * (uint64_t)i + ((!a.single && i >= 1) ? 2 : 0);
    const uint32_t q = a.q[src + i], t = a.t[src + i];
    const int len = a.len[src + i];
    const uint32_t lf = (uint32_t)(g - f0);
    a.fq[g] = q; a.ft[g] = t; a.flen[g] = len; a.fcl[g] = cl; a.fai[g] = i;
    a.fval[g] = len * rate;
    a.fprevNode[g] = NONE; a.fprevInd[g] = NONE; a.fflags[g] = 3; a.used[g] = 0; a.fstrand[g] = (uint8_t)(strand != 0);
    const bool edge = !a.single && (i == 0 || i == n - 1);
    for (int rep = 0; rep < (edge ? 2 : 1); rep++) {
      const int pair = (strand == 0) ? rep : 1 - rep;
      uint32_t sq, st, eq, et;
      if (pair == 0) { sq = q; st = t; eq = q + len; et = t + len; }
      else { sq = q; st = t + len; eq = q + len; et = t; }
      const uint8_t inv = pair == 0 ? 1 : 0;
      for (int e = 0; e < 2; e++, p++) {
        const uint32_t pq = e ? eq : sq, pt = e ? et : st;
        const uint8_t ind = e ? 0 : 1;
        a.key1[p] = ((uint64_t)pq << 33) | ((uint64_t)pt << 1) | ind;
        a.pay1[p] = (uint32_t)(p - p0);
        a.iq[p] = pq; a.it[p] = pt; a.ifl[p] = (uint8_t)(ind | (inv << 1)); a.ifr[p] = lf; a.ptRead[p] = r;
      }
    }
  }
}

__global__ void k_gather(uint64_t np, const uint32_t* __restrict__ ptRead, const uint64_t* __restrict__ ptOff, const uint32_t* __restrict__ pay1,
                         const uint32_t* __restrict__ iq, const uint32_t* __restrict__ it, const uint8_t* __restrict__ ifl,
                         const uint32_t* __restrict__ ifr, uint32_t* hq, uint32_t* ht, uint8_t* hfl, uint32_t* hfr, uint64_t* key2,
                         uint32_t* pay2, uint64_t* key3, uint32_t* pay3) {
  uint64_t p = (uint64_t)blockIdx.x * blockDim.x + threadIdx.x;
  if (p >= np) return;
  const uint64_t p0 = ptOff[ptRead[p]];
  const uint64_t s = p0 + pay1[p];
  const uint32_t q = iq[s], t = it[s];
  const uint8_t fl = ifl[s];
  hq[p] = q; ht[p] = t; hfl[p] = fl; hfr[p] = ifr[s];
  key2[p] = ((uint64_t)t << 31) | ((uint64_t)q << 1) | (fl & 1);
  pay2[p] = (uint32_t)(p - p0);
  const int inv = (fl >> 1) & 1, ind = fl & 1;
  const uint64_t cls = (uint64_t)((inv ? 0 : 2) + (ind ? 0 : 1));
  const uint64_t dg = inv ? (uint64_t)((int64_t)t - (int64_t)q + (1LL << 32)) : (uint64_t)t + q;
  key3[p] = (cls << 40) | dg;
  pay3[p] = (uint32_t)(p - p0);
}

__global__ void k_reset_frags(int r0, const uint32_t* __restrict__ order, const uint64_t* __restrict__ fragOff, const int32_t* __restrict__ flen,
                              const float* __restrict__ rate_in, float rate, float* fval, uint32_t* fprevNode, uint32_t* fprevInd, uint8_t* fflags,
                              uint32_t* status) {
  const int r = r0 + (int)order[blockIdx.x];
  const float rt = rate_in ? rate_in[r] : rate;
  for (uint64_t g = fragOff[r] + threadIdx.x; g < fragOff[r + 1]; g += blockDim.x) { fval[g] = flen[g] * rt; fprevNode[g] = NONE; fprevInd[g] = NONE; fflags[g] = 3; }
  if (threadIdx.x == 0) status[r] = 0;
}

__global__ void k_pen_table(PwlTab pw, int n, short* tab, int* bad) {
  const int d = blockIdx.x * blockDim.x + threadIdx.x;
  if (d >= n) return;
  const float w = pwl_w(pw.slope, pw.inter, pw.c1, pw.c2, 0, (long long)d);
  const float p = -w;
  if (!(p >= 0.f && p <= 32767.f) || (float)(int)p != p) { atomicOr(bad, 1); tab[d] = 0; return; }
  tab[d] = (short)(int)p;
}

__global__ void k_frag_read(int n_reads, const uint64_t* __restrict__ fragOff, uint32_t* fragRead) {
  int r = blockIdx.x;
  for (uint64_t g = fragOff[r] + threadIdx.x; g < fragOff[r + 1]; g += blockDim.x) fragRead[g] = r;
}

inline dim3 grid256(uint64_t n) { return dim3((unsigned)((n + 255) / 256)); }

}

namespace lra_sdp {

void launch_cluster_counts(hipStream_t st, uint64_t nc, const uint32_t* c_count, uint32_t* fragCnt, uint32_t* ptCnt, int single) {
  hipLaunchKernelGGL(k_cluster_counts, grid256(nc), dim3(256), 0, st, nc, c_count, fragCnt, ptCnt, single);
}
void launch_read_offsets(hipStream_t st, int n_reads, const uint64_t* cluster_off, const uint64_t* clusFragOff, const uint64_t* clusPtOff, uint64_t* fragOff, uint64_t* ptOff,
                         uint32_t* clusRead, uint32_t* status, uint32_t* nChains) {
  hipLaunchKernelGGL(k_read_offsets, grid256((uint64_t)n_reads + 1), dim3(256), 0, st, n_reads, cluster_off, clusFragOff, clusPtOff, fragOff, ptOff, clusRead, status, nChains);
}
void launch_points(hipStream_t st, const PtArgs& pa) {
  if (pa.qe) hipLaunchKernelGGL(k_points, dim3((unsigned)((pa.nc + 127) / 128)), dim3(128), 0, st, pa);
  else hipLaunchKernelGGL(k_points, dim3((unsigned)((pa.nc + 3) / 4)), dim3(256), 0, st, pa);
}
void launch_frag_read(hipStream_t st, int n_reads, const uint64_t* fragOff, uint32_t* fragRead) {
  hipLaunchKernelGGL(k_frag_read, dim3(n_reads), dim3(64), 0, st, n_reads, fragOff, fragRead);
}
void launch_gather(hipStream_t st, uint64_t np, const uint32_t* ptRead, const uint64_t* ptOff, const uint32_t* pay1, const uint32_t* iq, const uint32_t* it, const uint8_t* ifl,
                   const uint32_t* ifr, uint32_t* hq, uint32_t* ht, uint8_t* hfl, uint32_t* hfr, uint64_t* key2, uint32_t* pay2, uint64_t* key3, uint32_t* pay3) {
  hipLaunchKernelGGL(k_gather, grid256(np), dim3(256), 0, st, np, ptRead, ptOff, pay1, iq, it, ifl, ifr, hq, ht, hfl, hfr, key2, pay2, key3, pay3);
}
void launch_reset_frags(hipStream_t st, int n, int r0, const uint32_t* order, const uint64_t* fragOff, const int32_t* flen, const float* rate_in, float rate, float* fval,
                        uint32_t* fprevNode, uint32_t* fprevInd, uint8_t* fflags, uint32_t* status) {
  hipLaunchKernelGGL(k_reset_frags, dim3(n), dim3(64), 0, st, r0, order, fragOff, flen, rate_in, rate, fval, fprevNode, fprevInd, fflags, status);
}
void launch_pen_table(hipStream_t st, const PwlTab& pw, short* tab, int* bad) {
  hipLaunchKernelGGL(k_pen_table, dim3(PEN_TAB_WG / 256), dim3(256), 0, st, pw, PEN_TAB_WG, tab, bad);
}
void launch_arena_estimate(hipStream_t st, int n, int r0, const uint64_t* ptOff, float fE, float fN, uint32_t* cntE, uint32_t* cntN, uint32_t* cntD) {
  hipLaunchKernelGGL(k_arena_estimate, dim3((n + 255) / 256), dim3(256), 0, st, n, r0, ptOff, fE, fN, cntE, cntN, cntD);
}
void launch_arena_sizes(hipStream_t st, int n, int r0, const uint64_t* ptOff, const uint32_t* cntE, const uint32_t* cntN, const uint32_t* cntD, ReadArena* ra, uint64_t* bytes,
                        const uint32_t* order, int shift) {
  hipLaunchKernelGGL(k_arena_sizes, dim3((n + 255) / 256), dim3(256), 0, st, n, r0, ptOff, cntE, cntN, cntD, ra, bytes, order, shift);
}
void launch_arena_bases(hipStream_t st, int n, const uint64_t* byteOff, ReadArena* ra, const uint32_t* order, char* arena) {
  hipLaunchKernelGGL(k_arena_bases, dim3((n + 255) / 256), dim3(256), 0, st, n, byteOff, ra, order, arena);
}
void launch_visit_clear(hipStream_t st, int n, const ReadArena* ra, const uint64_t* byteOff, const uint32_t* order) {
  hipLaunchKernelGGL(k_visit_clear, dim3(n), dim3(256), 0, st, ra, byteOff, order);
}
void launch_big_lines(hipStream_t st, int n, int r0, const uint32_t* order, const uint64_t* ptOff, const uint32_t* hq, const uint32_t* ht, const uint32_t* h2, uint32_t* maxLines) {
  hipLaunchKernelGGL(k_big_lines, dim3(n), dim3(256), 0, st, r0, order, ptOff, hq, ht, h2, maxLines);
}

}
```

### lra_amd/csrc/sdp_process.hip

```cpp
#include "sdp_process.h"

using namespace lra_sdp;

namespace {

template <bool STAT>
__global__ void __launch_bounds__(64, 4) sdp_process(ProcArgs a) {
  __shared__ unsigned long long sT[STAT ? 10 : 1], sC[STAT ? 20 : 1];
  unsigned long long tPrev = 0;
  if (STAT) { if (threadIdx.x < 10) sT[threadIdx.x] = 0; if (threadIdx.x < 20) sC[threadIdx.x] = 0; tPrev = __builtin_amdgcn_s_memtime(); }
#define TICK(k_) do { if (STAT) { if (a.dbg == 2) __builtin_amdgcn_s_waitcnt(0); const unsigned long long t__ = __builtin_amdgcn_s_memtime(); if (threadIdx.x == 0) sT[k_] += t__ - tPrev; tPrev = t__; } } while (0)
#define CNT(k_, x_) do { const unsigned long long x__ = (unsigned long long)(x_); if (threadIdx.x == 0) sC[k_] += x__; } while (0)
#define WMAX(x_) ([&]() { int m__ = (x_); for (int o__ = 32; o__ > 0; o__ >>= 1) m__ = max(m__, __shfl_xor(m__, o__)); return m__; }())
  __shared__ float s_slope[25], s_inter[25];
  __shared__ short s_pen[PEN_TAB_WAVE];
  const int lane = threadIdx.x;
  if (lane < 25) { s_slope[lane] = a.pwl.slope[lane]; s_inter[lane] = a.pwl.inter[lane]; }
  const int penN = min(a.penN, PEN_TAB_WAVE);
  for (int x = lane; x < penN; x += 64) s_pen[x] = a.penTab[x];
  __syncthreads();
  const int c1 = a.pwl.c1, c2 = a.pwl.c2;
  const int rr = (int)a.order[blockIdx.x], r = a.r0 + rr;
  if (a.status[r] & LRA_ST_CAPACITY) return;
  const uint64_t p0 = a.ptOff[r], f0 = a.fragOff[r];
  const int P = (int)(a.ptOff[r + 1] - p0);
  const float rate = a.rate_in ? a.rate_in[r] : a.rate;
  const ReadArena A = a.ra[rr];
  char* ab = arena_ptr(A.base);
  Node* nodes = (Node*)ab;
  Ent* ent = (Ent*)(ab + A.entOff);
  uint32_t* Ap = (uint32_t*)(ab + A.apOff);
  const long long* Ed = (const long long*)(ab + A.edOff);
  int2* pairs = (int2*)(ab + A.stkOff);
  const uint32_t poolPair = A.poolPair, poolPairs = A.poolPairs;
  uint32_t* poolUsed = a.poolUsed + rr;
  const uint2* visR = (const uint2*)(ab + A.visOff);
  const int fam2 = lane < LV ? 0 : 1, level = lane < LV ? lane : lane - LV;
  uint32_t bad = 0;
  Node cn; cn.dBase = 0; cn.nD = 0; cn.nE = 0; cn.last = -1; cn.sTop = 0; cn.nBlk = 0; cn.stkOff = 0; cn.blkOff = 0; cn.stkCap = 0; cn.blkCap = 0;
  uint32_t cId = NONE;
  int2 cTop = make_int2(0, 0), cLastB = make_int2(0, 0);
  bool cTopOk = false, cDirty = false;
  int vz; asm volatile("v_mov_b32_e32 %0, 0" : "=v"(vz));
  uint32_t flN = P > 0 ? a.hfl[p0 + vz] : 0;
  uint32_t lfN = P > 0 ? a.hfr[p0 + vz] : 0;
  static_assert(sizeof(Node) == 48, "a descriptor is fetched as three 16-byte pieces");
  __shared__ uint4 s_node[2][3][2 * LV];
  uint2 vN = make_uint2(NONE, 0), vNN = make_uint2(NONE, 0);
  if (P > 0 && lane < 2 * LV) vN = visR[lane];
  if (P > 1 && lane < 2 * LV) vNN = visR[(uint64_t)(2 * LV) + lane];
#define NODE_FETCH(id_, buf_) do { const char* src__ = (const char*)(nodes + (id_)); _Pragma("unroll") for (int w__ = 0; w__ < 3; w__++) \
    __builtin_amdgcn_global_load_lds((const __attribute__((address_space(1))) void*)(src__ + 16 * w__), (__attribute__((address_space(3))) void*)&s_node[(buf_)][w__][0], 16, 0, 0); } while (0)
  if (vN.x != NONE) NODE_FETCH(vN.x, 0);
  for (int pi = 0; pi < P && !bad; pi++) {
    const uint8_t fl = (uint8_t)u_u(flN);
    const uint32_t lf = u_u(lfN);
    const uint2 v = vN;
    vN = vNN;
    bool swd = false;
    if (v.x != NONE && v.x != cId) {
      swd = true;
      const uint4 w0 = s_node[pi & 1][0][lane], w1 = s_node[pi & 1][1][lane], w2 = s_node[pi & 1][2][lane];
      if (cDirty) { Node* op = nodes + cId; op->last = cn.last; op->sTop = cn.sTop; op->nBlk = cn.nBlk; op->stkOff = cn.stkOff; op->stkCap = cn.stkCap; op->blkOff = cn.blkOff; op->blkCap = cn.blkCap; cDirty = false; }
      cn.dBase = w0.x; cn.nD = w0.y; cn.nE = w0.z; cn.last = (int32_t)w0.w; cn.sTop = w1.x; cn.nBlk = w1.y; cn.stkOff = w1.z; cn.blkOff = w1.w; cn.stkCap = w2.x; cn.blkCap = w2.y;
      cn.eLast = (long long)(((unsigned long long)w2.w << 32) | w2.z);
      cId = v.x; cTopOk = false;
    }
    if (pi + 1 < P) {
      vNN = make_uint2(NONE, 0);
      if (pi + 2 < P && lane < 2 * LV) vNN = visR[(uint64_t)(pi + 2) * (2 * LV) + lane];
      flN = a.hfl[p0 + pi + 1 + vz]; lfN = a.hfr[p0 + pi + 1 + vz];
    }
    if (vN.x != NONE && vN.x != cId) NODE_FETCH(vN.x, (pi + 1) & 1);
    const int ind = fl & 1, inv = (fl >> 1) & 1;
    const float fvP = a.fval[f0 + lf];
    if (STAT) { const int sw = __popcll(__ballot(swd)); const int nl = __popcll(__ballot(v.x != NONE)); CNT(ind ? 1 : 0, 1); CNT(ind ? 3 : 2, sw > 0); CNT(ind ? 5 : 4, nl); TICK(ind ? 1 : 0); }
    if (ind == 0) {
      if (v.x != NONE) {
        const float val = fvP;
        const uint32_t e = cn.dBase + v.y;
        if (ent[e].v < val) { ent[e].v = val; Ap[e] = lf; }
      }
      TICK(2);
    } else {
      const Node& nd = cn;
      int now = -1;
      long long ei1 = 0;
      const int m = (int)nd.nD, n = (int)nd.nE, i1 = (int)v.y;
      int sTop = (int)nd.sTop, nBlk = (int)nd.nBlk;
      uint32_t stkOff = nd.stkOff, blkOff = nd.blkOff;
      int sCap = (int)nd.stkCap, bCap = (int)nd.blkCap;
      const long long eLast = nd.eLast;
      int tx = cTop.x; int2 lastB = cLastB;
      constexpr int SX_UNK = -2;
      int sx = cTop.y;
      uint32_t st = 0;
      Ent pfD; pfD.val = 0; pfD.b = -1; pfD.v = 0;
      long long pfE = 0;
      Ent pfT; pfT.val = 0; pfT.b = 0; pfT.v = 0;
      bool pfTok = false;
      float pfSv = 0.f; long long pfSd = 0; int pfSx = SX_UNK;
      if (v.x != NONE) {
        const Ent e = ent[nd.dBase + nd.nD + v.y];
        int2 sT = make_int2(-1, 0), sS = make_int2(-1, 0), bL = make_int2(0, 0);
        if (!cTopOk) { if (sTop > 1) sT = (pairs + stkOff)[sTop - 1]; if (sTop > 2) sS = (pairs + stkOff)[sTop - 2]; if (nBlk > 0) bL = (pairs + blkOff)[nBlk - 1]; }
        if (nd.last + 1 < m) { pfD = (ent + nd.dBase)[nd.last + 1]; pfE = (Ed + nd.dBase)[nd.last + 1]; }
        if (cTopOk && tx >= 0) { pfT = (ent + nd.dBase)[tx]; pfTok = true; }
        if (cTopOk && sx >= 0) { const Ent es = (ent + nd.dBase)[sx]; pfSv = es.v; pfSd = es.val; pfSx = sx; }
        now = e.b; ei1 = e.val;
        if (!cTopOk) { tx = sTop <= 1 ? -1 : sT.x; sx = sTop <= 2 ? -1 : sS.x; lastB = bL; }
      }
      const bool need = now != -1;
      const int pfTx = pfTok ? tx : SX_UNK;
      const int nBlk0 = nBlk; const uint32_t blkOff0 = blkOff;
      TICK(3);
      const int LOCAL_MAX = 4;
      const bool small = need && now > nd.last && now - nd.last <= LOCAL_MAX;
      int nIt = 0, nPop = 0;
      if (small) {
        bool topD = false; float tDv = 0; long long tDi = 0;
#define SPUSHL(val_) do { const int2 v__ = (val_); if (sTop >= sCap) { if (!grow_pairs(pairs, stkOff, sCap, sTop, poolUsed, poolPair, poolPairs)) st |= LRA_ST_CAPACITY; } \
                          if (sTop < sCap) (pairs + stkOff)[sTop] = v__; sTop++; } while (0)
#define BPUSHL(val_) do { const int2 v__ = (val_); if (nBlk >= bCap) { if (!grow_pairs(pairs, blkOff, bCap, nBlk, poolUsed, poolPair, poolPairs)) st |= LRA_ST_CAPACITY; } \
                          if (nBlk < bCap) (pairs + blkOff)[nBlk] = v__; nBlk++; lastB = v__; } while (0)
        for (int i = nd.last + 1; i <= now && !st; ++i) {
          if (STAT) nIt++;
          Ent di_ = pfD; long long edb = pfE;
          if (i != nd.last + 1) { di_ = (ent + nd.dBase)[i]; edb = (Ed + nd.dBase)[i]; }
          const int db = di_.b;
          if (db == -1) break;
          const long long di = di_.val; const float dvi = di_.v;
          if (tx == -1) { BPUSHL(make_int2(-1, db)); SPUSHL(make_int2(i, n)); tx = i; sx = -1; tDv = dvi; tDi = di; topD = true; }
          if (!topD) { Ent e = pfT; if (!pfTok) e = (ent + nd.dBase)[tx]; tDv = e.v; tDi = e.val; topD = true; }
          if (BEATS(dvi, di, tDv, tDi, edb)) {
            if (nBlk > 0 && db > lastB.y) BPUSHL(make_int2(tx, db));
            const float sNew = dvi + W(di, eLast);
            int cx = tx; float cDv = tDv; long long cDi = tDi;
            while (sTop > 0) {
              if (cx < 0 || n < 1) { st |= LRA_ST_OOB_SLOT; break; }
              if (!(sNew > cDv + W(cDi, eLast))) break;
              sTop--;
              if (STAT) nPop++;
              if (sTop == 0) { st |= LRA_ST_OOB_SLOT; break; }
              cx = sTop - 1 == 0 ? -1 : sx != SX_UNK ? sx : (pairs + stkOff)[sTop - 1].x;
              sx = sTop - 1 <= 1 ? -1 : SX_UNK;
              if (cx == -1) break;
              if (cx == pfSx) { cDv = pfSv; cDi = pfSd; }
              else { const Ent ce = (ent + nd.dBase)[cx]; cDv = ce.v; cDi = ce.val; }
            }
            if (st) break;
            SPUSHL(make_int2(i, n)); sx = cx; tx = i; tDv = dvi; tDi = di; topD = true;
          }
        }
#undef SPUSHL
#undef BPUSHL
      }
      if (STAT) { const int mi = WMAX(nIt), mp = WMAX(nPop); CNT(6, mi); CNT(7, mp); CNT(8, mi > 0); TICK(4); }
      unsigned long long todo = __ballot(need && now > nd.last && !small);
      if (STAT) CNT(9, __popcll(todo));
      while (todo) {
        const int owner = __ffsll((long long)todo) - 1;
        todo &= todo - 1;
        const Ent* oD = ent + (uint32_t)rl_i((int)nd.dBase, owner);
        const long long* oEd = Ed + (uint32_t)rl_i((int)nd.dBase, owner);
        const int on = rl_i(n, owner);
        const long long oeLast = rl_ll(eLast, owner);
        const int olast = rl_i(nd.last, owner), onow = rl_i(now, owner);
        int oTop = rl_i(sTop, owner), oBlk = rl_i(nBlk, owner);
        uint32_t oStkOff = (uint32_t)rl_i((int)stkOff, owner), oBlkOff = (uint32_t)rl_i((int)blkOff, owner);
        int2* oS = pairs + oStkOff; int2* oB = pairs + oBlkOff;
        int oSCap = rl_i(sCap, owner), oBCap = rl_i(bCap, owner);
        int otx = rl_i(tx, owner), osx = rl_i(sx, owner); int2 olastB = make_int2(rl_i(lastB.x, owner), rl_i(lastB.y, owner));
        uint32_t ost = 0;
        bool topD = rl_i(pfTok ? 1 : 0, owner) != 0; float tDv = rl_f(pfT.v, owner); long long tDi = rl_ll(pfT.val, owner);
        bool stop = false;
        for (int i0 = olast + 1; i0 <= onow && !stop && !ost; i0 += 64) {
          const int j = i0 + lane;
          Ent dj; dj.val = 0; dj.b = -1; dj.v = 0;
          long long ej = 0;
          if (j <= onow) { dj = oD[j]; ej = oEd[j]; }
          const int nb = min(64, onow - i0 + 1);
          int t = 0;
          while (t < nb && !ost) {
            if (otx != -1) {
              if (!topD) { const Ent e = oD[otx]; tDv = e.v; tDi = e.val; topD = true; }
              bool evt = false;
              if (lane >= t && lane < nb) evt = dj.b == -1 || BEATS(dj.v, dj.val, tDv, tDi, ej);
              const unsigned long long em = __ballot(evt);
              if (!em) break;
              t = __ffsll((long long)em) - 1;
            }
            const int i = i0 + t;
            const int db = rl_i(dj.b, t);
            if (db == -1) { stop = true; break; }
            const long long di = rl_ll(dj.val, t), edb = rl_ll(ej, t);
            const float dvi = rl_f(dj.v, t);
            bool win = true;
            if (otx == -1) { BPUSH(make_int2(-1, db)); SPUSH(make_int2(i, on)); otx = i; osx = -1; tDv = dvi; tDi = di; topD = true; win = BEATS(dvi, di, tDv, tDi, edb); }
            if (win) {
              if (oBlk > 0 && db > olastB.y) BPUSH(make_int2(otx, db));
              const float sNew = dvi + W(di, oeLast);
              int cx = otx; float cDv = tDv; long long cDi = tDi;
              while (oTop > 0) {
                if (cx < 0 || on < 1) { ost |= LRA_ST_OOB_SLOT; break; }
                if (!(sNew > cDv + W(cDi, oeLast))) break;
                oTop--;
                if (oTop == 0) { ost |= LRA_ST_OOB_SLOT; break; }
                cx = oTop - 1 == 0 ? -1 : osx != SX_UNK ? osx : oS[oTop - 1].x;
                osx = oTop - 1 <= 1 ? -1 : SX_UNK;
                if (cx == -1) break;
                const Ent ce = oD[cx]; cDv = ce.v; cDi = ce.val;
              }
              if (ost) break;
              SPUSH(make_int2(i, on)); osx = cx; otx = i; tDv = dvi; tDi = di; topD = true;
            }
            t++;
          }
        }
        if (lane == owner) { sTop = oTop; nBlk = oBlk; tx = otx; sx = osx; lastB = olastB; st |= ost; stkOff = oStkOff; blkOff = oBlkOff; sCap = oSCap; bCap = oBCap; }
      }
      TICK(5);
      float ev = -1.f;
      bool got = false;
      int nFl = 0, nSr = 0, nLd = 0, nBs = 0, nCh = 0;
      if (need && !st) {
#define BPUSH2(val_) do { const int2 v__ = (val_); if (nBlk >= bCap) { if (!grow_pairs(pairs, blkOff, bCap, nBlk, poolUsed, poolPair, poolPairs)) st |= LRA_ST_CAPACITY; } \
                          if (nBlk < bCap) (pairs + blkOff)[nBlk] = v__; nBlk++; lastB = v__; } while (0)
        if (now == m - 1) {
          while (sTop > 1 && tx != -1 && !st) {
            if (STAT) nFl++;
            BPUSH2(make_int2(tx, n)); sTop--;
            tx = sTop - 1 == 0 ? -1 : sx != SX_UNK ? sx : (pairs + stkOff)[sTop - 1].x;
            sx = sTop - 1 <= 1 ? -1 : SX_UNK;
          }
        }
#undef BPUSH2
        int i2 = -1;
        if (!st && nBlk > 0) {
          if (i1 >= lastB.y) i2 = tx;
          else {
            if (STAT) { nBs = nBlk; nCh = (nBlk != nBlk0 || blkOff != blkOff0) ? 1 : 0; }
            int lo = 0, cnt = nBlk, bx = -1;
            while (cnt > 0) {
              if (STAT) nSr++;
              const int step = cnt >> 1, it = lo + step;
              const int cntT = cnt - step - 1, itT = it + 1 + (cntT >> 1), itF = lo + (step >> 1);
              const int2 pM = (pairs + blkOff)[it], pT = cntT > 0 ? (pairs + blkOff)[itT] : make_int2(0, 0), pF = step > 0 ? (pairs + blkOff)[itF] : make_int2(0, 0);
              if (i1 >= pM.y) {
                lo = it + 1; cnt = cntT;
                if (cnt > 0) { const int s2 = cnt >> 1; if (i1 >= pT.y) { lo = itT + 1; cnt -= s2 + 1; } else { cnt = s2; bx = pT.x; } }
              } else {
                cnt = step; bx = pM.x;
                if (cnt > 0) { const int s2 = cnt >> 1; if (i1 >= pF.y) { lo = itF + 1; cnt -= s2 + 1; } else { cnt = s2; bx = pF.x; } }
              }
            }
            if (lo < nBlk) i2 = bx;
          }
        }
        if (st || i2 < 0 || i2 >= m) st |= st ? st : LRA_ST_OOB_SLOT;
        else {
          Ent d2;
          if (i2 == pfTx) d2 = pfT;
          else if (i2 == pfSx) { d2.v = pfSv; d2.val = pfSd; d2.b = 0; }
          else { d2 = (ent + nd.dBase)[i2]; if (STAT) nLd = 1; }
          ev = d2.v + W(d2.val, ei1) + rate * a.flen[f0 + lf];
          got = true;
          Ap[nd.dBase + nd.nD + i1] = (uint32_t)i2;
          cDirty = true;
          cn.last = now; cn.sTop = (uint32_t)sTop; cn.nBlk = (uint32_t)nBlk; cn.stkOff = stkOff; cn.blkOff = blkOff; cn.stkCap = (uint32_t)sCap; cn.blkCap = (uint32_t)bCap;
          cTop = make_int2(tx, sx); cLastB = lastB; cTopOk = true;
        }
      }
      if (STAT) { const int mf = WMAX(nFl), ms = WMAX(nSr), ml = WMAX(nLd), mb = WMAX(nBs), mc = WMAX(nCh), m2 = WMAX(nIt >= 2 ? 1 : 0); CNT(10, mf); CNT(11, ms); CNT(12, ml); CNT(13, ms > 0); CNT(14, mc); CNT(15, mb); CNT(16, m2); TICK(6); }
      const uint32_t myI1 = v.y;
      if (__ballot(st != 0)) { for (int o = 32; o > 0; o >>= 1) st |= __shfl_xor(st, o); }
      bad |= st;
      if (!bad) {
        const float bvM = wave_max_f32(got ? ev : -__builtin_inff());
        const unsigned long long eq = __ballot(got && ev == bvM);
        const unsigned long long eqR = eq & ((1ull << LV) - 1);
        const int win = eq ? 63 - __clzll((long long)(eqR ? eqR : eq)) : -1;
        if (lane == win) {
          if (fvP < ev) {
            a.fval[f0 + lf] = ev; a.fprevNode[f0 + lf] = v.x; a.fprevInd[f0 + lf] = myI1;
            a.fflags[f0 + lf] = (uint8_t)((fam2 == 0 ? 1 : 0) | (inv ? 2 : 0));
          }
        }
      }
      TICK(7);
    }
    wave_sync();
    TICK(ind ? 9 : 8);
  }
  if (STAT && lane == 0 && a.stat) { for (int k = 0; k < 10; k++) atomicAdd(a.stat + k, sT[k]); for (int k = 0; k < 20; k++) atomicAdd(a.stat + 10 + k, sC[k]); }
  if (cDirty && cId != NONE) { Node* op = nodes + cId; op->last = cn.last; op->sTop = cn.sTop; op->nBlk = cn.nBlk; op->stkOff = cn.stkOff; op->stkCap = cn.stkCap; op->blkOff = cn.blkOff; op->blkCap = cn.blkCap; }
  if (lane == 0 && bad) atomicOr(&a.status[r], bad);
#undef NODE_FETCH
#undef TICK
#undef CNT
#undef WMAX
}

}

namespace lra_sdp {

void launch_process(hipStream_t st, const ProcArgs& pa, int n, bool stat) {
  if (stat) hipLaunchKernelGGL(sdp_process<true>, dim3(n), dim3(64), 0, st, pa);
  else hipLaunchKernelGGL(sdp_process<false>, dim3(n), dim3(64), 0, st, pa);
}

}
```

### lra_amd/csrc/sdp_process_wg.hip

```cpp
#include "sdp_process.h"

using namespace lra_sdp;

namespace {

struct SlotState {
  Node cn; uint32_t cId; int dirty;
  int2 cTop, cLastB; int cTopOk;
  int topInfoOk, topDvOk; float topDv, topWe; long long topDi;
  int2 sec; int secOk, secDvOk; float secDv, secWe; long long secDi;
};
constexpr int WG_NW = 16;
constexpr int RING_W = 2048, RING_LEAD = 1024, RING_CHECK = 32;

__device__ __forceinline__ int wg_slot(int wave, int k) {
  static_assert(LV == 18 && WG_NW == 16, "slot table written for 18 levels on 16 waves");
  if (k == 0) return wave;
  if (k == 1) return LV + (15 - wave);
  return wave == 0 ? 16 : wave == 1 ? 17 : wave == 15 ? LV + 16 : wave == 14 ? LV + 17 : 2 * LV;
}

template <int SPW, bool DBG>
__global__ void __launch_bounds__(64 * WG_NW) sdp_process_wg(ProcArgs a) {
  __shared__ float s_slope[25], s_inter[25];
  __shared__ SlotState ss[2 * LV];
  __shared__ short s_pen[PEN_TAB_WG];
  __shared__ unsigned long long r_best[2 * RING_W];
  __shared__ uint32_t r_cnt[2 * RING_W];
  __shared__ int s_pos[WG_NW]; __shared__ uint32_t s_span, s_wtot[WG_NW];
  __shared__ uint32_t s_bad;
#define BAD() __hip_atomic_load(&s_bad, __ATOMIC_RELAXED, __HIP_MEMORY_SCOPE_WORKGROUP)
  const int tid = threadIdx.x, lane = tid & 63, wave = u_i(tid >> 6);
  if (tid < 25) { s_slope[tid] = a.pwl.slope[tid]; s_inter[tid] = a.pwl.inter[tid]; }
  const int penN = min(a.penN, PEN_TAB_WG);
  for (int x = tid; x < penN; x += 64 * WG_NW) s_pen[x] = a.penTab[x];
  if (tid < 2 * LV) {
    SlotState z; memset(&z, 0, sizeof z); z.cn.last = -1; z.cId = NONE;
    ss[tid] = z;
  }
  if (tid == 0) { s_bad = 0; s_span = 0; }
  if (tid < WG_NW) s_pos[tid] = 0;
  for (int x = tid; x < 2 * RING_W; x += 64 * WG_NW) { r_best[x] = 0; r_cnt[x] = 0; }
  __syncthreads();
  const int c1 = a.pwl.c1, c2 = a.pwl.c2;
  const int rr = (int)a.order[blockIdx.x], r = a.r0 + rr;
  if (a.status[r] & LRA_ST_CAPACITY) return;
  const uint64_t p0 = a.ptOff[r], f0 = a.fragOff[r];
  const int P = (int)(a.ptOff[r + 1] - p0);
  const float rate = a.rate_in ? a.rate_in[r] : a.rate;
  const ReadArena A = a.ra[rr];
  char* ab = arena_ptr(A.base);
  Node* nodes = (Node*)ab;
  Ent* ent = (Ent*)(ab + A.entOff);
  uint32_t* Ap = (uint32_t*)(ab + A.apOff);
  const long long* Ed = (const long long*)(ab + A.edOff);
  int2* pairs = (int2*)(ab + A.stkOff);
  const uint32_t poolPair = A.poolPair, poolPairs = A.poolPairs;
  uint32_t* poolUsed = a.poolUsed + rr;
  const uint2* visR = (const uint2*)(ab + A.visOff);
  const int F = (int)(a.fragOff[r + 1] - f0);
  char* wsb = a.wgScratch + a.wgOff[blockIdx.x];
  unsigned long long* best = (unsigned long long*)wsb;
  uint32_t* cnt = (uint32_t*)(wsb + 16 * (size_t)F);
  uint32_t* nS = cnt + 2 * (size_t)F;
  uint32_t* sPos = nS + F;
  uint32_t* pm = sPos + 2 * (size_t)F;
  for (int f = tid; f < F; f += 64 * WG_NW) { best[2 * f] = 0; best[2 * f + 1] = 0; cnt[2 * f] = 0; cnt[2 * f + 1] = 0; nS[f] = 0; sPos[2 * f] = 0; sPos[2 * f + 1] = 0; }
  __syncthreads();
  for (int pi = tid; pi < P; pi += 64 * WG_NW) {
    const uint32_t lf = a.hfr[p0 + pi];
    if (a.hfl[p0 + pi] & 1) { const uint32_t k = atomicAdd(&nS[lf], 1u); if (k < 2) sPos[2 * lf + k] = (uint32_t)pi; else atomicOr(&s_bad, (uint32_t)LRA_ST_RANGE); }
    else atomicMax(&cnt[2 * lf], (uint32_t)pi);
  }
  __syncthreads();
  for (int f = tid; f < F; f += 64 * WG_NW) {
    if (nS[f] == 2 && sPos[2 * f] > sPos[2 * f + 1]) { const uint32_t t = sPos[2 * f]; sPos[2 * f] = sPos[2 * f + 1]; sPos[2 * f + 1] = t; }
    if (nS[f] > 0 && cnt[2 * f] > sPos[2 * f]) atomicMax(&s_span, cnt[2 * f] - sPos[2 * f]);
    cnt[2 * f] = 0;
  }
  __syncthreads();
  const bool ring = a.wgNoRing == 0 && s_span + RING_LEAD + RING_CHECK + 1 <= (uint32_t)RING_W;
  if (ring) {
    const int per = (P + 64 * WG_NW - 1) / (64 * WG_NW), b0 = min(P, tid * per), b1 = min(P, b0 + per);
    uint32_t mine = 0;
    for (int pi = b0; pi < b1; pi++) mine += (a.hfl[p0 + pi] & 1) && sPos[2 * a.hfr[p0 + pi]] == (uint32_t)pi;
    uint32_t inc = mine;
    for (int o = 1; o < 64; o <<= 1) { const uint32_t t = __shfl_up(inc, o); if (lane >= o) inc += t; }
    if (lane == 63) s_wtot[wave] = inc;
    __syncthreads();
    uint32_t at = inc - mine;
    for (int w = 0; w < wave; w++) at += s_wtot[w];
    for (int pi = b0; pi < b1; pi++) { const uint32_t lf = a.hfr[p0 + pi]; if ((a.hfl[p0 + pi] & 1) && sPos[2 * lf] == (uint32_t)pi) cnt[2 * lf] = at++; }
    __syncthreads();
  }
  for (int pi = tid; pi < P; pi += 64 * WG_NW) {
    const uint32_t lf = a.hfr[p0 + pi];
    uint32_t k = 0;
    for (uint32_t x = 0; x < min(nS[lf], 2u); x++) k += sPos[2 * lf + x] < (uint32_t)pi;
    pm[pi] = ring ? (cnt[2 * lf] << 3) | (nS[lf] == 1 ? 4u : 0u) | k : k;
  }
  __threadfence();
  __syncthreads();
  unsigned long long* dbgT = (unsigned long long*)(((uintptr_t)(pm + P) + 7) & ~(uintptr_t)7);
  unsigned long long tRounds = 0, tEvents = 0, tStore = 0, tEvA = 0, tEvB = 0, tEvC = 0, tSwitch = 0, tDep = 0, tPub = 0;
  unsigned long long tSlot[4] = {0, 0, 0, 0}, tSec[4] = {0, 0, 0, 0};
  static_assert(SPW == 2 || SPW == (2 * LV + WG_NW - 1) / WG_NW, "slots per wave");
  uint2 vN[SPW]; uint32_t flN = P > 0 ? u_u(a.hfl[p0]) : 0, lfN = P > 0 ? u_u(a.hfr[p0]) : 0, rkN = P > 0 ? u_u(pm[0]) : 0;
#pragma unroll
  for (int k = 0; k < SPW; k++) { const int slot = wg_slot(wave, k); vN[k] = (P > 0 && slot < 2 * LV) ? u_u2(visR[slot]) : make_uint2(NONE, 0); }
  uint2 vV[SPW]; uint32_t lfV = 0, rkV = 0; uint8_t flV = 0;
#pragma unroll
  for (int k = 0; k < SPW; k++) vV[k] = make_uint2(NONE, 0);
  if (P > 1) {
    flV = a.hfl[p0 + 1]; lfV = a.hfr[p0 + 1]; rkV = pm[1];
#pragma unroll
    for (int k = 0; k < SPW; k++) { const int slot = wg_slot(wave, k); if (slot < 2 * LV) vV[k] = visR[(uint64_t)(2 * LV) + slot]; }
  }
  uint32_t ndV[SPW], pfId[SPW]; float fvV = 0.f;
#pragma unroll
  for (int k = 0; k < SPW; k++) { ndV[k] = 0; pfId[k] = NONE; }
  if (P > 0) fvV = a.fval[f0 + lfN];
  constexpr int NODE_WORDS = (int)(sizeof(Node) / 4);
  static_assert(sizeof(Node) % 4 == 0 && NODE_WORDS <= 64 && offsetof(SlotState, cn) == 0, "a descriptor is moved a word per lane");
  const unsigned long long tAll0 = DBG ? clock64() : 0;
  for (int pi = 0; pi < P && !BAD(); pi++) {
    const uint32_t fl = flN, lf = lfN, rk = rkN & 3u;
    const uint32_t re = 2 * ((rkN >> 3) & (uint32_t)(RING_W - 1)), gen = (rkN >> 3) / (uint32_t)RING_W + 1, single = (rkN >> 2) & 1u;
    const float fvC = fvV;
    const unsigned long long tp0 = DBG ? clock64() : 0;
    if (ring && (pi & (RING_CHECK - 1)) == 0 && lane == 0) {
      __hip_atomic_store(&s_pos[wave], pi, __ATOMIC_RELAXED, __HIP_MEMORY_SCOPE_WORKGROUP);
      for (;;) {
        int mn = pi;
        for (int w = 0; w < WG_NW; w++) mn = min(mn, __hip_atomic_load(&s_pos[w], __ATOMIC_RELAXED, __HIP_MEMORY_SCOPE_WORKGROUP));
        if (pi - mn <= RING_LEAD || BAD()) break;
        __builtin_amdgcn_s_sleep(8);
      }
    }
    uint2 vv[SPW]; Ent e0[SPW];
#pragma unroll
    for (int k = 0; k < SPW; k++) vv[k] = vN[k];
    const int ind = fl & 1;
    bool act[SPW];
#pragma unroll
    for (int k = 0; k < SPW; k++) {
      const int slot = wg_slot(wave, k);
      act[k] = slot < 2 * LV && vv[k].x != NONE;
      if (act[k] && vv[k].x != u_u(ss[slot].cId)) {
        SlotState& Zs = ss[slot];
        if (lane == 0 && Zs.dirty) { Node* op = nodes + Zs.cId; op->last = Zs.cn.last; op->sTop = Zs.cn.sTop; op->nBlk = Zs.cn.nBlk; op->stkOff = Zs.cn.stkOff; op->stkCap = Zs.cn.stkCap; op->blkOff = Zs.cn.blkOff; op->blkCap = Zs.cn.blkCap; Zs.dirty = 0; }
        uint32_t w = ndV[k];
        if (pfId[k] != vv[k].x && lane < NODE_WORDS) w = ((const uint32_t*)(nodes + vv[k].x))[lane];
        if (lane < NODE_WORDS) ((uint32_t*)&Zs)[lane] = w;
        if (lane == 0) { Zs.cId = vv[k].x; Zs.cTopOk = 0; Zs.topInfoOk = 0; Zs.topDvOk = 0; Zs.secOk = 0; Zs.secDvOk = 0; }
      }
    }
    wave_sync();
    if (pi + 1 < P) {
      flN = u_u(flV); lfN = u_u(lfV); rkN = u_u(rkV);
#pragma unroll
      for (int k = 0; k < SPW; k++) vN[k] = u_u2(vV[k]);
      if (pi + 2 < P) {
        flV = a.hfl[p0 + pi + 2]; lfV = a.hfr[p0 + pi + 2]; rkV = pm[pi + 2];
#pragma unroll
        for (int k = 0; k < SPW; k++) { const int slot = wg_slot(wave, k); if (slot < 2 * LV) vV[k] = visR[(uint64_t)(pi + 2) * (2 * LV) + slot]; }
      }
#pragma unroll
      for (int k = 0; k < SPW; k++) {
        const int slot = wg_slot(wave, k);
        pfId[k] = NONE;
        if (slot < 2 * LV && vN[k].x != NONE && vN[k].x != u_u(ss[slot].cId)) {
          pfId[k] = vN[k].x;
          if (lane < NODE_WORDS) ndV[k] = ((const uint32_t*)(nodes + vN[k].x))[lane];
        }
      }
      if (!(flN & 1)) fvV = a.fval[f0 + lfN];
    }
    if (DBG) { __builtin_amdgcn_s_waitcnt(0); tSwitch += clock64() - tp0; }
    float depVal = 0.f;
    if (!ind) {
      bool any = false;
#pragma unroll
      for (int k = 0; k < SPW; k++) any |= act[k];
      if (!any) continue;
      const unsigned long long tw0 = DBG ? clock64() : 0;
      if (lane == 0) {
        const int need = (int)rk;
        depVal = fvC;
        for (int x = 0; x < need; x++) {
          if (ring) {
            if (DBG) { tStore += 1ull << 32; if (__hip_atomic_load(&r_cnt[re + x], __ATOMIC_RELAXED, __HIP_MEMORY_SCOPE_WORKGROUP) < (uint32_t)WG_NW * gen) tStore++; }
            while (__hip_atomic_load(&r_cnt[re + x], __ATOMIC_RELAXED, __HIP_MEMORY_SCOPE_WORKGROUP) < (uint32_t)WG_NW * gen && !BAD()) __builtin_amdgcn_s_sleep(2);
            const unsigned long long key = __hip_atomic_load(&r_best[re + x], __ATOMIC_RELAXED, __HIP_MEMORY_SCOPE_WORKGROUP);
            const float v = __uint_as_float((uint32_t)(key >> 16));
            if ((uint32_t)(key >> 48) == gen && depVal < v) depVal = v;
          } else {
            if (DBG) { tStore += 1ull << 32; if (__hip_atomic_load(&cnt[2 * lf + x], __ATOMIC_RELAXED, __HIP_MEMORY_SCOPE_AGENT) < (uint32_t)WG_NW) tStore++; }
            while (__hip_atomic_load(&cnt[2 * lf + x], __ATOMIC_RELAXED, __HIP_MEMORY_SCOPE_AGENT) < (uint32_t)WG_NW && !BAD()) __builtin_amdgcn_s_sleep(2);
            const unsigned long long key = __hip_atomic_load(&best[2 * lf + x], __ATOMIC_RELAXED, __HIP_MEMORY_SCOPE_AGENT);
            const float v = __uint_as_float((uint32_t)(key >> 32));
            if (key && depVal < v) depVal = v;
          }
        }
      }
      if (DBG) tSlot[3] += clock64() - tw0;
    }
    if (ind) {
#pragma unroll
      for (int k = 0; k < SPW; k++) {
        e0[k].b = -1; e0[k].val = 0; e0[k].v = 0;
        if (act[k]) { const Node& nd = ss[wg_slot(wave, k)].cn; e0[k] = ent[u_u(nd.dBase) + u_u(nd.nD) + vv[k].y]; }
      }
    }
    float wBest = -2.f; int wRank = 0;
#pragma unroll 1
    for (int k = 0; k < SPW; k++) {
      const int slot = wg_slot(wave, k);
      if (slot >= 2 * LV) continue;
      const uint2 v = k == 0 ? vv[0] : k == 1 ? vv[1] : vv[SPW - 1];
      const Ent e0k = k == 0 ? e0[0] : k == 1 ? e0[1] : e0[SPW - 1];
      if (!(k == 0 ? act[0] : k == 1 ? act[1] : act[SPW - 1])) continue;
      const unsigned long long ts0 = DBG ? clock64() : 0;
      SlotState& Z = ss[slot];
      Node nd;
      { const Node& zn = Z.cn; nd.dBase = u_u(zn.dBase); nd.nD = u_u(zn.nD); nd.nE = u_u(zn.nE); nd.last = u_i(zn.last); nd.sTop = u_u(zn.sTop); nd.nBlk = u_u(zn.nBlk); nd.stkOff = u_u(zn.stkOff);
        nd.blkOff = u_u(zn.blkOff); nd.stkCap = u_u(zn.stkCap); nd.blkCap = u_u(zn.blkCap); nd.eLast = u_ll(zn.eLast); }
      if (ind == 0) {
        if (lane == 0) {
          const float val = depVal;
          const uint32_t e = nd.dBase + v.y;
          if (ent[e].v < val) {
            ent[e].v = val; Ap[e] = lf;
            if (Z.cTopOk && Z.cTop.x == (int)v.y) Z.topDvOk = 0;
            if (Z.cTopOk && Z.secOk && Z.sec.x == (int)v.y) Z.secDvOk = 0;
          }
        }
        if (DBG) { __builtin_amdgcn_s_waitcnt(0); tDep += clock64() - ts0; }
        continue;
      }
      const int now = u_i(e0k.b);
      const long long ei1 = u_ll(e0k.val);
      const bool need = now != -1;
      const int m = (int)nd.nD, n = (int)nd.nE, i1 = (int)v.y;
      int oTop = (int)nd.sTop, oBlk = (int)nd.nBlk;
      uint32_t oStkOff = nd.stkOff, oBlkOff = nd.blkOff;
      int2* oS = pairs + oStkOff; int2* oB = pairs + oBlkOff;
      int oSCap = (int)nd.stkCap, oBCap = (int)nd.blkCap;
      const Ent* oD = ent + nd.dBase;
      const long long* oEd = Ed + nd.dBase;
      const long long eLast = nd.eLast;
      uint32_t ost = 0;
      const int on = n;
      int tx = -1, sx = -1; int2 olastB = make_int2(0, 0);
      bool tInfo = false, tDvOk = false, secOk = false, sInfo = false, sDvOk = false;
      float tDv = 0.f, tWe = 0.f, sDv = 0.f, sWe = 0.f; long long tDi = 0, sDi = 0;
      if (need) {
        if (u_i(Z.cTopOk)) {
          tx = u_i(Z.cTop.x); olastB = u_i2(Z.cLastB); tInfo = u_i(Z.topInfoOk) != 0; tDvOk = u_i(Z.topDvOk) != 0; tDv = u_f(Z.topDv); tDi = u_ll(Z.topDi); tWe = u_f(Z.topWe);
          secOk = u_i(Z.secOk) != 0; sx = u_i(Z.sec.x); sInfo = secOk; sDi = u_ll(Z.secDi); sWe = u_f(Z.secWe); sDvOk = u_i(Z.secDvOk) != 0; sDv = u_f(Z.secDv);
        } else if (oTop > 0) { tx = oTop == 1 ? -1 : u_i(oS[oTop - 1].x); olastB = oBlk > 0 ? u_i2(oB[oBlk - 1]) : make_int2(0, 0); }
      }
#define PAIR_INFO(x_, di_, dv_, we_) do { const Ent d__ = oD[(x_)]; (di_) = u_ll(d__.val); (dv_) = u_f(d__.v); (we_) = W((di_), eLast); } while (0)
#define NEXT_DOWN(x_, infoOk_, di_, we_, dv_, dvOk_) do { if (secOk) { (x_) = sx; (di_) = sDi; (we_) = sWe; (infoOk_) = true; (dv_) = sDv; (dvOk_) = sDvOk; secOk = false; sDvOk = false; } \
                                               else if (oTop - 1 == 0) { (x_) = -1; (infoOk_) = true; (dvOk_) = false; } \
                                               else { (x_) = u_i(oS[oTop - 1].x); (infoOk_) = false; (dvOk_) = false; } } while (0)
      unsigned long long tq = 0;
      if (DBG) { __builtin_amdgcn_s_waitcnt(0); tq = clock64(); tSec[0] += tq - ts0; }
      if (need && now > nd.last) {
        const int olast = nd.last, onow = now;
        bool stop = false;
        for (int i0 = olast + 1; i0 <= onow && !stop && !ost; i0 += 64) {
          const int j = i0 + lane;
          Ent dj; dj.val = 0; dj.b = -1; dj.v = 0;
          long long ej = 0;
          const unsigned long long tl0 = DBG ? clock64() : 0;
          if (j <= onow) { dj = oD[j]; ej = oEd[j]; }
          if (DBG) { __builtin_amdgcn_s_waitcnt(0); tSlot[2] += clock64() - tl0; tRounds++; }
          const int nb = min(64, onow - i0 + 1);
          int t = 0;
          while (t < nb && !ost) {
            const unsigned long long te0 = DBG ? clock64() : 0;
            if (tx != -1) {
              if (!tInfo) { PAIR_INFO(tx, tDi, tDv, tWe); tInfo = true; tDvOk = true; }
              else if (!tDvOk) { tDv = u_f(oD[tx].v); tDvOk = true; }
              bool evt = false;
              if (lane >= t && lane < nb) evt = dj.b == -1 || BEATS(dj.v, dj.val, tDv, tDi, ej);
              const unsigned long long em = __ballot(evt);
              if (!em) break;
              t = __ffsll((long long)em) - 1;
            }
            const int i = i0 + t;
            const int db = rl_i(dj.b, t);
            if (db == -1) { stop = true; break; }
            unsigned long long te1 = 0;
            if (DBG) { tEvents++; te1 = clock64(); tEvA += te1 - te0; }
            const long long di = rl_ll(dj.val, t), edb = rl_ll(ej, t);
            const float dvi = rl_f(dj.v, t);
            bool win = true;
            if (tx == -1) {
              BPUSH(make_int2(-1, db)); SPUSH(make_int2(i, on));
              sx = -1; secOk = true; sInfo = true; sDvOk = false;
              tx = i; tDv = dvi; tDi = di; tWe = W(di, eLast); tInfo = true; tDvOk = true;
              win = BEATS(dvi, di, tDv, tDi, edb);
            }
            unsigned long long te2 = 0;
            if (DBG) { te2 = clock64(); tEvB += te2 - te1; }
            if (win) {
              if (oBlk > 0 && db > olastB.y) BPUSH(make_int2(tx, db));
              const float wNew = W(di, eLast), sNew = dvi + wNew;
              int cx = tx; float cDv = tDv, cWe = tWe; long long cDi = tDi; bool cInfo = true, cDvOk = true;
              while (oTop > 0) {
                if (cx < 0 || on < 1) { ost |= LRA_ST_OOB_SLOT; break; }
                if (!(sNew > cDv + cWe)) break;
                oTop--;
                if (oTop == 0) { ost |= LRA_ST_OOB_SLOT; break; }
                NEXT_DOWN(cx, cInfo, cDi, cWe, cDv, cDvOk);
                if (cx == -1) break;
                if (!cInfo) { PAIR_INFO(cx, cDi, cDv, cWe); cInfo = true; cDvOk = true; }
                else if (!cDvOk) { cDv = u_f(oD[cx].v); cDvOk = true; }
              }
              if (ost) break;
              SPUSH(make_int2(i, on));
              sx = cx; secOk = cx == -1 || cInfo; sInfo = secOk; sDi = cDi; sWe = cWe; sDv = cDv; sDvOk = cx != -1 && cInfo && cDvOk;
              tx = i; tDv = dvi; tDi = di; tWe = wNew; tInfo = true; tDvOk = true;
            }
            if (DBG) tEvC += clock64() - te2;
            t++;
          }
        }
      }
      float ev = -2.f;
      if (DBG) { __builtin_amdgcn_s_waitcnt(0); const unsigned long long t1 = clock64(); tSec[1] += t1 - tq; tq = t1; }
      if (need && !ost) {
        if (now == m - 1) { while (oTop > 1 && tx != -1 && !ost) { BPUSH(make_int2(tx, on)); oTop--; NEXT_DOWN(tx, tInfo, tDi, tWe, tDv, tDvOk); } }
        int i2 = -1;
        if (!ost && oBlk > 0) {
          if (i1 >= olastB.y) i2 = tx;
          else {
            int bx;
            const unsigned lo = coop_upper_block(oB, (unsigned)oBlk, i1, lane, &bx);
            if ((int)lo < oBlk) i2 = bx;
          }
        }
        if (DBG) { __builtin_amdgcn_s_waitcnt(0); const unsigned long long t1 = clock64(); tSec[2] += t1 - tq; tq = t1; }
        if (ost || i2 < 0 || i2 >= m) ost |= ost ? ost : LRA_ST_OOB_SLOT;
        else {
          float d2v; long long d2d;
          if (i2 == tx && tInfo && tDvOk) { d2v = tDv; d2d = tDi; }
          else { const Ent d2 = oD[i2]; d2v = u_f(d2.v); d2d = u_ll(d2.val); if (i2 == tx && tInfo) { tDv = d2v; tDvOk = true; } }
          ev = u_f(d2v + W(d2d, ei1) + rate * a.flen[f0 + lf]);
          if (lane == 0) {
            Ap[nd.dBase + nd.nD + i1] = (uint32_t)i2;
            Z.dirty = 1;
            Z.cn.last = now; Z.cn.sTop = (uint32_t)oTop; Z.cn.nBlk = (uint32_t)oBlk; Z.cn.stkOff = oStkOff; Z.cn.blkOff = oBlkOff; Z.cn.stkCap = (uint32_t)oSCap; Z.cn.blkCap = (uint32_t)oBCap;
            Z.cTop = make_int2(tx, tx == -1 ? on + 1 : on); Z.cLastB = olastB; Z.cTopOk = 1;
            Z.topInfoOk = tInfo ? 1 : 0; Z.topDvOk = (tInfo && tDvOk) ? 1 : 0; Z.topDv = tDv; Z.topDi = tDi; Z.topWe = tWe;
            Z.secOk = (secOk && sInfo) ? 1 : 0; Z.sec = make_int2(sx, sx == -1 ? on + 1 : on); Z.secDi = sDi; Z.secWe = sWe; Z.secDv = sDv; Z.secDvOk = (secOk && sInfo && sDvOk) ? 1 : 0;
          }
        }
      }
#undef PAIR_INFO
#undef NEXT_DOWN
      if (ost && lane == 0) atomicOr(&s_bad, ost);
      const int vr = (slot / LV) * LV + (LV - 1 - slot % LV);
      if (ev > 0.f && (ev > wBest || (ev == wBest && vr < wRank))) { wBest = ev; wRank = vr; }
      if (DBG) { __builtin_amdgcn_s_waitcnt(0); const unsigned long long t1 = clock64(); if (k == 0) tSlot[0] += t1 - ts0; else if (k == 1) tSlot[1] += t1 - ts0; else tSlot[2] += t1 - ts0; tSec[3] += t1 - tq; }
    }
    wave_sync();
    const unsigned long long tb0 = DBG ? clock64() : 0;
    if (ind && lane == 0) {
      const int x = (int)rk;
      if (ring) {
        if (wBest > 0.f) (void)__hip_atomic_fetch_max(&r_best[re + x], ((unsigned long long)gen << 48) | ((unsigned long long)__float_as_uint(wBest) << 16) | (unsigned long long)(0xFFFFu - (uint32_t)wRank),
                                                      __ATOMIC_RELAXED, __HIP_MEMORY_SCOPE_WORKGROUP);
        const uint32_t was = __hip_atomic_fetch_add(&r_cnt[re + x], 1u, __ATOMIC_RELAXED, __HIP_MEMORY_SCOPE_WORKGROUP);
        if (single) (void)__hip_atomic_fetch_add(&r_cnt[re + 1], 1u, __ATOMIC_RELAXED, __HIP_MEMORY_SCOPE_WORKGROUP);
        if (was + 1 == (uint32_t)WG_NW * gen) {
          const unsigned long long key = __hip_atomic_load(&r_best[re + x], __ATOMIC_RELAXED, __HIP_MEMORY_SCOPE_WORKGROUP);
          if ((uint32_t)(key >> 48) == gen) best[2 * lf + x] = ((key >> 16) & 0xFFFFFFFFull) << 32 | (unsigned long long)(0xFFFFFFFFu - (0xFFFFu - (uint32_t)(key & 0xFFFFu)));
        }
      } else {
      uint32_t one = 1u;
      if (wBest > 0.f) {
        const unsigned long long was = __hip_atomic_fetch_max(&best[2 * lf + x], ((unsigned long long)__float_as_uint(wBest) << 32) | (unsigned long long)(0xFFFFFFFFu - (uint32_t)wRank),
                                                              __ATOMIC_RELAXED, __HIP_MEMORY_SCOPE_AGENT);
        one += (uint32_t)(was == 0xFFFFFFFFFFFFFFFFull);
      }
      (void)__hip_atomic_fetch_add(&cnt[2 * lf + x], one, __ATOMIC_RELAXED, __HIP_MEMORY_SCOPE_AGENT);
      }
    }
    if (DBG) { __builtin_amdgcn_s_waitcnt(0); tPub += clock64() - tb0; }
  }
  if (DBG && lane == 0) {
    unsigned long long* o = dbgT + 16 * wave;
    o[0] = clock64() - tAll0; o[1] = tSlot[3]; o[2] = tSwitch; o[3] = tDep; o[4] = tPub; o[5] = tSec[0]; o[6] = tSec[1]; o[7] = tSec[2]; o[8] = tSec[3];
    o[9] = tEvA; o[10] = tEvB; o[11] = tEvC; o[12] = (tRounds << 32) | tEvents; o[13] = tStore; o[14] = tSlot[0] + tSlot[1] + tSlot[2]; o[15] = 0;
  }
  __syncthreads();
  if (!s_bad) {
    for (int f = tid; f < F; f += 64 * WG_NW) {
      float val = a.fval[f0 + f];
      int win = -1; unsigned long long wkey = 0;
      for (uint32_t x = 0; x < min(nS[f], 2u); x++) {
        const unsigned long long key = best[2 * f + x];
        const float v = __uint_as_float((uint32_t)(key >> 32));
        if (key && val < v) { val = v; win = (int)x; wkey = key; }
      }
      if (win >= 0) {
        const int vr = (int)(0xFFFFFFFFu - (uint32_t)wkey);
        const int slot = (vr / LV) * LV + (LV - 1 - vr % LV);
        const uint32_t pi = sPos[2 * f + win];
        const uint2 v = visR[(uint64_t)pi * (2 * LV) + slot];
        a.fval[f0 + f] = val; a.fprevNode[f0 + f] = v.x; a.fprevInd[f0 + f] = v.y;
        a.fflags[f0 + f] = (uint8_t)((slot < LV ? 1 : 0) | (((a.hfl[p0 + pi] >> 1) & 1) ? 2 : 0));
      }
    }
  }
  if (tid == 0 && s_bad) atomicOr(&a.status[r], (uint32_t)s_bad);
#undef BAD
}

}

namespace lra_sdp {

void launch_process_wg(hipStream_t st, const ProcArgs& pa, int n, uint32_t lines, bool dbg) {
  if (lines <= 32768) { if (dbg) hipLaunchKernelGGL((sdp_process_wg<2, true>), dim3(n), dim3(64 * WG_NW), 0, st, pa); else hipLaunchKernelGGL((sdp_process_wg<2, false>), dim3(n), dim3(64 * WG_NW), 0, st, pa); }
  else { if (dbg) hipLaunchKernelGGL((sdp_process_wg<3, true>), dim3(n), dim3(64 * WG_NW), 0, st, pa); else hipLaunchKernelGGL((sdp_process_wg<3, false>), dim3(n), dim3(64 * WG_NW), 0, st, pa); }
}

}
```

Before: 1.140.

## Store visit records plane-major and size planes by per-read line counts

The per-point visit table changes from a point-major array of 2*LV slots to level planes, each laid out contiguously over points. Only as many planes as the tree depth implied by the row and column line counts are allocated. Line counts are now recorded by the count pass and the big-lines kernel, then used to size the arena. This shrinks arena memory, cuts the visit-clear traffic, and makes per-lane loads in the process kernels stride by point within a plane. The build kernel's level limit now depends on the computed plane count, so an underestimate of the needed depth would be reported as a range overflow.

```diff
diff --git a/lra_amd/csrc/sdp.h b/lra_amd/csrc/sdp.h
--- a/lra_amd/csrc/sdp.h
+++ b/lra_amd/csrc/sdp.h
@@ -23,7 +23,7 @@
   long long eLast;
 };
 
-struct ReadArena { uint64_t base; uint32_t entOff, apOff, stkOff, visOff, blkPair, poolPair, poolPairs, edOff; };
+struct ReadArena { uint64_t base; uint32_t entOff, apOff, stkOff, visOff, blkPair, poolPair, poolPairs, edOff, visPl; };
 
 struct PtArgs {
   uint64_t nc;
@@ -44,6 +44,7 @@
   const uint32_t* hq; const uint32_t* ht; const uint8_t* hfl; const uint32_t* h2; const uint64_t* key3; const uint32_t* pay3;
   uint32_t* scratch;
   uint32_t* cntEntries; uint32_t* cntNodes; uint32_t* cntD; uint32_t* cntV; uint32_t* cntRC;
+  uint32_t* lines;
   const ReadArena* ra;
   uint32_t* status;
   unsigned long long* stat;
@@ -98,6 +99,17 @@
   return v;
 }
 __device__ __host__ inline uint32_t al256(uint64_t x) { return (uint32_t)((x + 255) & ~(uint64_t)255); }
+__device__ __host__ inline uint32_t vis_planes(uint64_t n) {
+  uint32_t d = 1;
+  while (d < (uint32_t)LV && (uint64_t(1) << (d - 1)) < n) d++;
+  return d;
+}
+__device__ __forceinline__ uint32_t vis_plane(uint32_t visPl, int slot) {
+  const uint32_t plR = visPl & 0xffu, plC = visPl >> 8;
+  if (slot < LV) return (uint32_t)slot < plR ? (uint32_t)slot : NONE;
+  const uint32_t lv = (uint32_t)(slot - LV);
+  return lv < plC ? plR + lv : NONE;
+}
 __device__ __forceinline__ char* arena_ptr(uint64_t addr) { return (char*)(__attribute__((address_space(1))) char*)addr; }
 }
 
@@ -134,6 +146,7 @@
 struct Chunk {
   int r0, r1, nr; uint64_t cp;
   uint32_t* scratch; uint32_t* cntE; uint32_t* cntN; uint32_t* cntD; uint32_t* cntV; uint32_t* cntRC; uint32_t* order; uint32_t* order2; uint32_t* poolUsed;
+  uint32_t* lines;
   uint64_t* bytes; uint64_t* byteOff; ReadArena* ra;
   std::vector<uint32_t> h_orderAll, h_prev;
   BuildArgs ba; StatBuf buildStat;
@@ -167,11 +180,12 @@
                         uint32_t* fprevNode, uint32_t* fprevInd, uint8_t* fflags, uint32_t* status);
 void launch_pen_table(hipStream_t st, const PwlTab& pw, short* tab, int* bad);
 void launch_arena_estimate(hipStream_t st, int n, int r0, const uint64_t* ptOff, float fE, float fN, uint32_t* cntE, uint32_t* cntN, uint32_t* cntD);
-void launch_arena_sizes(hipStream_t st, int n, int r0, const uint64_t* ptOff, const uint32_t* cntE, const uint32_t* cntN, const uint32_t* cntD, ReadArena* ra, uint64_t* bytes,
-                        const uint32_t* order, int shift);
+void launch_arena_sizes(hipStream_t st, int n, int r0, const uint64_t* ptOff, const uint32_t* cntE, const uint32_t* cntN, const uint32_t* cntD, const uint32_t* lines, ReadArena* ra,
+                        uint64_t* bytes, const uint32_t* order, int shift);
 void launch_arena_bases(hipStream_t st, int n, const uint64_t* byteOff, ReadArena* ra, const uint32_t* order, char* arena);
 void launch_visit_clear(hipStream_t st, int n, const ReadArena* ra, const uint64_t* byteOff, const uint32_t* order);
-void launch_big_lines(hipStream_t st, int n, int r0, const uint32_t* order, const uint64_t* ptOff, const uint32_t* hq, const uint32_t* ht, const uint32_t* h2, uint32_t* maxLines);
+void launch_big_lines(hipStream_t st, int n, int r0, const uint32_t* order, const uint64_t* ptOff, const uint32_t* hq, const uint32_t* ht, const uint32_t* h2, uint32_t* maxLines,
+                      uint32_t* lines);
 void launch_wg_builds(bool emit, hipStream_t st, const BuildArgs& ba, int n);
 void launch_small_builds(bool emit, lra_ctx* ctx, const BuildArgs& ba, const uint32_t* d_order, const std::vector<uint32_t>& h_order, const uint64_t* h_pt, int from, int to);
 void launch_process(hipStream_t st, const ProcArgs& pa, int n, bool stat);
diff --git a/lra_amd/csrc/sdp.hip b/lra_amd/csrc/sdp.hip
--- a/lra_amd/csrc/sdp.hip
+++ b/lra_amd/csrc/sdp.hip
@@ -147,12 +147,14 @@
   lra_ctx* ctx = c.ctx; hipStream_t st = c.st; const std::vector<uint64_t>& h_pt = c.h_pt;
   const int r0 = k.r0, nr = k.nr; const uint64_t cp = k.cp;
   const size_t nr1 = (size_t)nr + 1;
-  size_t needS = sz(34 * cp + 64 * (size_t)nr + 64, 4) + sz(nr1, 4) * 8 + sz(nr1 + 1, 8) * 3 + sz(nr1, sizeof(ReadArena)) + 4096;
+  size_t needS = sz(34 * cp + 64 * (size_t)nr + 64, 4) + sz(nr1, 4) * 8 + sz(2 * nr1, 4) + sz(nr1 + 1, 8) * 3 + sz(nr1, sizeof(ReadArena)) + 4096;
   char* ws = (char*)lra_ensure(ctx, 10, needS);
   if (!ws) return LRA_ERR_NOMEM;
   k.scratch = (uint32_t*)take(ws, 34 * cp + 64 * (size_t)nr + 64, 4);
   k.cntE = (uint32_t*)take(ws, nr1, 4); k.cntN = (uint32_t*)take(ws, nr1, 4); k.cntD = (uint32_t*)take(ws, nr1, 4);
   k.cntV = (uint32_t*)take(ws, nr1, 4); k.cntRC = (uint32_t*)take(ws, nr1, 4); k.order = (uint32_t*)take(ws, nr1, 4); k.order2 = (uint32_t*)take(ws, nr1, 4); k.poolUsed = (uint32_t*)take(ws, nr1, 4);
+  k.lines = (uint32_t*)take(ws, 2 * nr1, 4);
+  LRA_HIP_CHECK(ctx, hipMemsetAsync(k.lines, 0, 2 * nr1 * 4, st));
   {
     std::vector<uint32_t> h_order(nr);
     uint64_t maxP = 0;
@@ -179,7 +181,7 @@
   BuildArgs& ba = k.ba;
   memset(&ba, 0, sizeof ba);
   ba.r0 = r0; ba.n = nr; ba.ptOff = c.ptOff; ba.hq = c.hq; ba.ht = c.ht; ba.hfl = c.hfl; ba.h2 = c.pay2; ba.key3 = c.key1; ba.pay3 = c.pay1; ba.scratch = k.scratch;
-  ba.cntEntries = k.cntE; ba.cntNodes = k.cntN; ba.cntD = k.cntD; ba.cntV = k.cntV; ba.cntRC = k.cntRC; ba.status = c.status; ba.order = k.order; ba.stat = nullptr;
+  ba.cntEntries = k.cntE; ba.cntNodes = k.cntN; ba.cntD = k.cntD; ba.cntV = k.cntV; ba.cntRC = k.cntRC; ba.lines = k.lines; ba.status = c.status; ba.order = k.order; ba.stat = nullptr;
   if (diag_build_stat()) { k.buildStat.alloc(16, st); ba.stat = k.buildStat.d; }
   k.h_status.assign(nr, 0);
   k.subOrder = k.order; k.nsub = nr;
@@ -260,10 +262,10 @@
     LRA_HIP_CHECK(ctx, hipMemcpyAsync(a.dwoff, woff.data(), ((size_t)nbig + 1) * 8, hipMemcpyHostToDevice, st));
     if (a.early) {
       LRA_HIP_CHECK(ctx, hipMemsetAsync(a.d_maxLines, 0, 4, st));
-      launch_big_lines(st, nbig, r0, k.subOrder, c.ptOff, c.hq, c.ht, c.pay2, a.d_maxLines);
+      launch_big_lines(st, nbig, r0, k.subOrder, c.ptOff, c.hq, c.ht, c.pay2, a.d_maxLines, k.lines);
     }
   }
-  launch_arena_sizes(st, nsub, r0, c.ptOff, k.cntE, k.cntN, k.cntD, k.ra, k.bytes, k.subOrder, a.shift);
+  launch_arena_sizes(st, nsub, r0, c.ptOff, k.cntE, k.cntN, k.cntD, k.lines, k.ra, k.bytes, k.subOrder, a.shift);
   SDP_TRY(lra_exclusive_scan<uint64_t>(ctx, nsub, k.bytes, k.byteOff));
   LRA_HIP_CHECK(ctx, hipMemcpyAsync(&a.totB, k.byteOff + nsub, 8, hipMemcpyDeviceToHost, st));
   if (a.early) LRA_HIP_CHECK(ctx, hipMemcpyAsync(&a.bigLines, a.d_maxLines, 4, hipMemcpyDeviceToHost, st));
diff --git a/lra_amd/csrc/sdp_build.hip b/lra_amd/csrc/sdp_build.hip
--- a/lra_amd/csrc/sdp_build.hip
+++ b/lra_amd/csrc/sdp_build.hip
@@ -90,11 +90,11 @@
   BTICK(0);
   uint32_t nEntries = 0, nNodesTot = 0, sumD = 0, nVisits = 0;
   Node* nodesR = nullptr; Ent* entR = nullptr; uint32_t* apR = nullptr; int2* stkR = nullptr; uint2* visR = nullptr; long long* edR = nullptr;
-  uint32_t blkPair = 0;
+  uint32_t blkPair = 0, visPl = 0;
   if (EMIT) {
     const ReadArena A = a.ra[rr];
     char* b = arena_ptr(A.base);
-    blkPair = A.blkPair;
+    blkPair = A.blkPair; visPl = A.visPl;
     nodesR = (Node*)b; entR = (Ent*)(b + A.entOff); apR = (uint32_t*)(b + A.apOff); stkR = (int2*)(b + A.stkOff); visR = (uint2*)(b + A.visOff);
     edR = (long long*)(b + A.edOff);
   }
@@ -108,6 +108,8 @@
     const int nS = cOff[sc + 1] - cOff[sc], nEn = cOff[sc + 2] - cOff[sc + 1], Pf = nS + nEn;
     if (nS == 0 || nEn == 0) continue;
     const int fam2 = fam & 1;
+    const int nPl = EMIT ? (int)(fam2 ? visPl >> 8 : visPl & 0xffu) : LV;
+    uint2* visF = EMIT ? visR + (size_t)(fam2 ? visPl & 0xffu : 0u) * P : nullptr;
     const int dSide = swapped ? 1 : 0, eSide = swapped ? 0 : 1;
     for (int i = tid; i < Pf; i += NT) {
       const uint32_t pos = pay3[cOff[sc] + i];
@@ -119,7 +121,8 @@
     SYNC();
     BTICK(7);
     for (int level = 0; nNodes > 0 && !outgrown; level++) {
-      if (level >= LV) { overflow = true; break; }
+      if (level >= nPl) { overflow = true; break; }
+      uint2* visL = EMIT ? visF + (size_t)level * P : nullptr;
       const int nxt = cur ^ 1;
       IT* lpc = lp + cur * P; IT* lpn = lp + nxt * P;
       IT* llc = ll + cur * P; IT* lln = ll + nxt * P;
@@ -350,7 +353,7 @@
                   entR[ent].val = dgv;
                   if (isS && idx == n - 1) nodesR[gid].eLast = dgv;
                 }
-                visR[(uint64_t)pos * (2 * LV) + fam2 * LV + level] = make_uint2(gid, idx);
+                visL[pos] = make_uint2(gid, idx);
               }
             }
           }
@@ -458,7 +461,7 @@
     for (int w = 0; w < NW; w++) nVisits += (uint32_t)s_w[0][w];
   }
   if (tid == 0) {
-    if (!EMIT) { a.cntEntries[rr] = nEntries; a.cntNodes[rr] = nNodesTot; a.cntD[rr] = sumD; a.cntV[rr] = nVisits; a.cntRC[rr] = (uint32_t)max(R, C); }
+    if (!EMIT) { a.cntEntries[rr] = nEntries; a.cntNodes[rr] = nNodesTot; a.cntD[rr] = sumD; a.cntV[rr] = nVisits; a.cntRC[rr] = (uint32_t)max(R, C); a.lines[2 * rr] = (uint32_t)R; a.lines[2 * rr + 1] = (uint32_t)C; }
     else { a.cntV[rr] = nEntries; a.cntRC[rr] = (uint32_t)max(R, C); }
     if (overflow) atomicOr(&a.status[r], (uint32_t)LRA_ST_RANGE);
     if (outgrown) atomicOr(&a.status[r], (uint32_t)LRA_ST_CAPACITY);
diff --git a/lra_amd/csrc/sdp_points.hip b/lra_amd/csrc/sdp_points.hip
--- a/lra_amd/csrc/sdp_points.hip
+++ b/lra_amd/csrc/sdp_points.hip
@@ -6,7 +6,8 @@
 namespace {
 
 __global__ void k_arena_sizes(int n, int r0, const uint64_t* __restrict__ ptOff, const uint32_t* __restrict__ cntE, const uint32_t* __restrict__ cntN,
-                              const uint32_t* __restrict__ cntD, ReadArena* ra, uint64_t* bytes, const uint32_t* __restrict__ order, int shift) {
+                              const uint32_t* __restrict__ cntD, const uint32_t* __restrict__ lines, ReadArena* ra, uint64_t* bytes,
+                              const uint32_t* __restrict__ order, int shift) {
   int b = blockIdx.x * blockDim.x + threadIdx.x;
   if (b >= n) return;
   const int rr = (int)order[b];
@@ -20,7 +21,10 @@
   const uint64_t stkPairs = 2 * D + 4 * N + 2, blkPairs = 2 * E + 8 * N + 2, poolPairs = (2 * E + 4096) << shift;
   a.stkOff = (uint32_t)o; a.blkPair = (uint32_t)stkPairs; a.poolPair = (uint32_t)(stkPairs + blkPairs); a.poolPairs = (uint32_t)poolPairs;
   o = al256(o + (stkPairs + blkPairs + poolPairs) * 8);
-  a.visOff = (uint32_t)o; o = al256(o + P * 2 * LV * sizeof(uint2));
+  const uint32_t nR = lines[2 * rr], nC = lines[2 * rr + 1];
+  const uint32_t plR = vis_planes(nR ? nR : P), plC = vis_planes(nC ? nC : P);
+  a.visPl = plR | (plC << 8);
+  a.visOff = (uint32_t)o; o = al256(o + P * (plR + plC) * sizeof(uint2));
   ra[rr] = a;
   bytes[b] = o;
 }
@@ -44,8 +48,8 @@
 }
 
 __global__ void k_big_lines(int r0, const uint32_t* __restrict__ order, const uint64_t* __restrict__ ptOff, const uint32_t* __restrict__ hq, const uint32_t* __restrict__ ht,
-                            const uint32_t* __restrict__ h2, uint32_t* maxLines) {
-  const int r = r0 + (int)order[blockIdx.x];
+                            const uint32_t* __restrict__ h2, uint32_t* maxLines, uint32_t* lines) {
+  const int rr = (int)order[blockIdx.x], r = r0 + rr;
   const uint64_t p0 = ptOff[r];
   const int P = (int)(ptOff[r + 1] - p0);
   const uint32_t* q = hq + p0; const uint32_t* t = ht + p0; const uint32_t* c = h2 + p0;
@@ -57,7 +61,7 @@
   __syncthreads();
   if ((threadIdx.x & 63) == 0) { atomicAdd(&sR, R); atomicAdd(&sC, C); }
   __syncthreads();
-  if (threadIdx.x == 0) atomicMax(maxLines, max(sR, sC));
+  if (threadIdx.x == 0) { atomicMax(maxLines, max(sR, sC)); lines[2 * rr] = sR; lines[2 * rr + 1] = sC; }
 }
 
 __global__ void k_cluster_counts(uint64_t nc, const uint32_t* __restrict__ c_count, uint32_t* fragCnt, uint32_t* ptCnt, int single) {
@@ -217,9 +221,9 @@
 void launch_arena_estimate(hipStream_t st, int n, int r0, const uint64_t* ptOff, float fE, float fN, uint32_t* cntE, uint32_t* cntN, uint32_t* cntD) {
   hipLaunchKernelGGL(k_arena_estimate, dim3((n + 255) / 256), dim3(256), 0, st, n, r0, ptOff, fE, fN, cntE, cntN, cntD);
 }
-void launch_arena_sizes(hipStream_t st, int n, int r0, const uint64_t* ptOff, const uint32_t* cntE, const uint32_t* cntN, const uint32_t* cntD, ReadArena* ra, uint64_t* bytes,
-                        const uint32_t* order, int shift) {
-  hipLaunchKernelGGL(k_arena_sizes, dim3((n + 255) / 256), dim3(256), 0, st, n, r0, ptOff, cntE, cntN, cntD, ra, bytes, order, shift);
+void launch_arena_sizes(hipStream_t st, int n, int r0, const uint64_t* ptOff, const uint32_t* cntE, const uint32_t* cntN, const uint32_t* cntD, const uint32_t* lines, ReadArena* ra,
+                        uint64_t* bytes, const uint32_t* order, int shift) {
+  hipLaunchKernelGGL(k_arena_sizes, dim3((n + 255) / 256), dim3(256), 0, st, n, r0, ptOff, cntE, cntN, cntD, lines, ra, bytes, order, shift);
 }
 void launch_arena_bases(hipStream_t st, int n, const uint64_t* byteOff, ReadArena* ra, const uint32_t* order, char* arena) {
   hipLaunchKernelGGL(k_arena_bases, dim3((n + 255) / 256), dim3(256), 0, st, n, byteOff, ra, order, arena);
@@ -227,8 +231,9 @@
 void launch_visit_clear(hipStream_t st, int n, const ReadArena* ra, const uint64_t* byteOff, const uint32_t* order) {
   hipLaunchKernelGGL(k_visit_clear, dim3(n), dim3(256), 0, st, ra, byteOff, order);
 }
-void launch_big_lines(hipStream_t st, int n, int r0, const uint32_t* order, const uint64_t* ptOff, const uint32_t* hq, const uint32_t* ht, const uint32_t* h2, uint32_t* maxLines) {
-  hipLaunchKernelGGL(k_big_lines, dim3(n), dim3(256), 0, st, r0, order, ptOff, hq, ht, h2, maxLines);
-}
-
-}
+void launch_big_lines(hipStream_t st, int n, int r0, const uint32_t* order, const uint64_t* ptOff, const uint32_t* hq, const uint32_t* ht, const uint32_t* h2, uint32_t* maxLines,
+                      uint32_t* lines) {
+  hipLaunchKernelGGL(k_big_lines, dim3(n), dim3(256), 0, st, r0, order, ptOff, hq, ht, h2, maxLines, lines);
+}
+
+}
diff --git a/lra_amd/csrc/sdp_process.hip b/lra_amd/csrc/sdp_process.hip
--- a/lra_amd/csrc/sdp_process.hip
+++ b/lra_amd/csrc/sdp_process.hip
@@ -36,6 +36,8 @@
   uint32_t* poolUsed = a.poolUsed + rr;
   const uint2* visR = (const uint2*)(ab + A.visOff);
   const int fam2 = lane < LV ? 0 : 1, level = lane < LV ? lane : lane - LV;
+  const uint32_t visPlane = vis_plane(A.visPl, lane);
+  const uint32_t visAt = visPlane != NONE ? visPlane * (uint32_t)P : NONE;
   uint32_t bad = 0;
   Node cn; cn.dBase = 0; cn.nD = 0; cn.nE = 0; cn.last = -1; cn.sTop = 0; cn.nBlk = 0; cn.stkOff = 0; cn.blkOff = 0; cn.stkCap = 0; cn.blkCap = 0;
   uint32_t cId = NONE;
@@ -47,8 +49,8 @@
   static_assert(sizeof(Node) == 48, "a descriptor is fetched as three 16-byte pieces");
   __shared__ uint4 s_node[2][3][2 * LV];
   uint2 vN = make_uint2(NONE, 0), vNN = make_uint2(NONE, 0);
-  if (P > 0 && lane < 2 * LV) vN = visR[lane];
-  if (P > 1 && lane < 2 * LV) vNN = visR[(uint64_t)(2 * LV) + lane];
+  if (P > 0 && visAt != NONE) vN = visR[visAt];
+  if (P > 1 && visAt != NONE) vNN = visR[visAt + 1u];
 #define NODE_FETCH(id_, buf_) do { const char* src__ = (const char*)(nodes + (id_)); _Pragma("unroll") for (int w__ = 0; w__ < 3; w__++) \
     __builtin_amdgcn_global_load_lds((const __attribute__((address_space(1))) void*)(src__ + 16 * w__), (__attribute__((address_space(3))) void*)&s_node[(buf_)][w__][0], 16, 0, 0); } while (0)
   if (vN.x != NONE) NODE_FETCH(vN.x, 0);
@@ -68,7 +70,7 @@
     }
     if (pi + 1 < P) {
       vNN = make_uint2(NONE, 0);
-      if (pi + 2 < P && lane < 2 * LV) vNN = visR[(uint64_t)(pi + 2) * (2 * LV) + lane];
+      if (pi + 2 < P && visAt != NONE) vNN = visR[visAt + (uint32_t)(pi + 2)];
       flN = a.hfl[p0 + pi + 1 + vz]; lfN = a.hfr[p0 + pi + 1 + vz];
     }
     if (vN.x != NONE && vN.x != cId) NODE_FETCH(vN.x, (pi + 1) & 1);
diff --git a/lra_amd/csrc/sdp_process_wg.hip b/lra_amd/csrc/sdp_process_wg.hip
--- a/lra_amd/csrc/sdp_process_wg.hip
+++ b/lra_amd/csrc/sdp_process_wg.hip
@@ -106,15 +106,21 @@
   unsigned long long tSlot[4] = {0, 0, 0, 0}, tSec[4] = {0, 0, 0, 0};
   static_assert(SPW == 2 || SPW == (2 * LV + WG_NW - 1) / WG_NW, "slots per wave");
   uint2 vN[SPW]; uint32_t flN = P > 0 ? u_u(a.hfl[p0]) : 0, lfN = P > 0 ? u_u(a.hfr[p0]) : 0, rkN = P > 0 ? u_u(pm[0]) : 0;
-#pragma unroll
-  for (int k = 0; k < SPW; k++) { const int slot = wg_slot(wave, k); vN[k] = (P > 0 && slot < 2 * LV) ? u_u2(visR[slot]) : make_uint2(NONE, 0); }
+  uint32_t visAt[SPW];
+#pragma unroll
+  for (int k = 0; k < SPW; k++) {
+    const int slot = wg_slot(wave, k);
+    const uint32_t pl = slot < 2 * LV ? vis_plane(A.visPl, slot) : NONE;
+    visAt[k] = pl != NONE ? pl * (uint32_t)P : NONE;
+    vN[k] = (P > 0 && visAt[k] != NONE) ? u_u2(visR[visAt[k]]) : make_uint2(NONE, 0);
+  }
   uint2 vV[SPW]; uint32_t lfV = 0, rkV = 0; uint8_t flV = 0;
 #pragma unroll
   for (int k = 0; k < SPW; k++) vV[k] = make_uint2(NONE, 0);
   if (P > 1) {
     flV = a.hfl[p0 + 1]; lfV = a.hfr[p0 + 1]; rkV = pm[1];
 #pragma unroll
-    for (int k = 0; k < SPW; k++) { const int slot = wg_slot(wave, k); if (slot < 2 * LV) vV[k] = visR[(uint64_t)(2 * LV) + slot]; }
+    for (int k = 0; k < SPW; k++) if (visAt[k] != NONE) vV[k] = visR[visAt[k] + 1u];
   }
   uint32_t ndV[SPW], pfId[SPW]; float fvV = 0.f;
 #pragma unroll
@@ -163,7 +169,7 @@
       if (pi + 2 < P) {
         flV = a.hfl[p0 + pi + 2]; lfV = a.hfr[p0 + pi + 2]; rkV = pm[pi + 2];
 #pragma unroll
-        for (int k = 0; k < SPW; k++) { const int slot = wg_slot(wave, k); if (slot < 2 * LV) vV[k] = visR[(uint64_t)(pi + 2) * (2 * LV) + slot]; }
+        for (int k = 0; k < SPW; k++) if (visAt[k] != NONE) vV[k] = visR[visAt[k] + (uint32_t)(pi + 2)];
       }
 #pragma unroll
       for (int k = 0; k < SPW; k++) {
@@ -410,7 +416,7 @@
         const int vr = (int)(0xFFFFFFFFu - (uint32_t)wkey);
         const int slot = (vr / LV) * LV + (LV - 1 - vr % LV);
         const uint32_t pi = sPos[2 * f + win];
-        const uint2 v = visR[(uint64_t)pi * (2 * LV) + slot];
+        const uint2 v = visR[(uint64_t)vis_plane(A.visPl, slot) * (uint32_t)P + pi];
         a.fval[f0 + f] = val; a.fprevNode[f0 + f] = v.x; a.fprevInd[f0 + f] = v.y;
         a.fflags[f0 + f] = (uint8_t)((slot < LV ? 1 : 0) | (((a.hfl[p0 + pi] >> 1) & 1) ? 2 : 0));
       }
```

After: 1.160, median of 6. +1.7%, better.
